# OliBomby/Mapperatorinator

Measured on NVIDIA H100. Metric: event tokens/sec end-to-end (mel+T5+DiT), higher is better.
Workload: dtype f32

## Files before the change

mapperatorinator_b200/csrc/attention.cu:

```cuda
#include "common.cuh"
#include "kernels.h"

namespace mb200 {
namespace {

constexpr int TQ = 64, TK = 64, HD = 64, LDS_ = 68;

__device__ __forceinline__ bool mask_allowed(const AttentionParams& p, int b, int q, int k) {
    if (k >= p.Tk) return false;
    if (p.key_valid && !p.key_valid[(long long)b * p.key_valid_ld + k]) return false;
    switch (p.mask_mode) {
        case MASK_CAUSAL: return k <= p.q_pos0 + q;
        case MASK_BAND:   return (q >= k - p.band) && (q < k + p.band);
        case MASK_DENSE:  return q < p.Tq && !p.dense[(long long)q * p.Tk + k];
        default:          return true;
    }
}

__global__ void __launch_bounds__(256) attention_kernel(AttentionParams p) {
    extern __shared__ __align__(16) float smem[];
    float (*Qt)[LDS_] = reinterpret_cast<float (*)[LDS_]>(smem);
    float (*Kt)[LDS_] = reinterpret_cast<float (*)[LDS_]>(smem + HD * LDS_);
    float (*Vs)[LDS_] = reinterpret_cast<float (*)[LDS_]>(smem + 2 * HD * LDS_);
    float (*Ps)[LDS_] = reinterpret_cast<float (*)[LDS_]>(smem + 3 * HD * LDS_);

    const int tid = threadIdx.x, tx = tid & 15, ty = tid >> 4;
    const int q0 = blockIdx.x * TQ, h = blockIdx.y, b = blockIdx.z;
    const float* qb = p.q + (long long)b * p.q_bs + h * HD;
    const int kvb = p.kv_slot ? p.kv_slot[b] : b;
    const float* kb = p.k + (long long)kvb * p.k_bs + h * HD;
    const float* vb = p.v + (long long)kvb * p.v_bs + h * HD;

    {
        const int r = tid >> 4, dq = (tid & 15) * 4;
#pragma unroll
        for (int rr = 0; rr < 4; ++rr) {
            int row = r + rr * 16, q = q0 + row;
            float4 v = q < p.Tq ? *reinterpret_cast<const float4*>(qb + (long long)q * p.q_ld + dq) : make_float4(0, 0, 0, 0);
            Qt[dq + 0][row] = v.x * p.scale; Qt[dq + 1][row] = v.y * p.scale;
            Qt[dq + 2][row] = v.z * p.scale; Qt[dq + 3][row] = v.w * p.scale;
        }
    }

    int kt_begin = 0, kt_end = (p.Tk + TK - 1) / TK;
    if (p.mask_mode == MASK_CAUSAL) {
        int last = p.q_pos0 + min(q0 + TQ - 1, p.Tq - 1);
        kt_end = min(kt_end, last / TK + 1);
    } else if (p.mask_mode == MASK_BAND) {
        int lo = q0 - p.band + 1, hi = min(q0 + TQ - 1, p.Tq - 1) + p.band;
        kt_begin = max(0, lo) / TK;
        kt_end = min(kt_end, hi / TK + 1);
    }

    float m_i[4], l_i[4], o[4][4];
#pragma unroll
    for (int i = 0; i < 4; ++i) {
        m_i[i] = -INFINITY; l_i[i] = 0.f;
#pragma unroll
        for (int j = 0; j < 4; ++j) o[i][j] = 0.f;
    }

    for (int kt = kt_begin; kt < kt_end; ++kt) {
        const int k0 = kt * TK;
        __syncthreads();
        {
            const int r = tid >> 4, dq = (tid & 15) * 4;
#pragma unroll
            for (int rr = 0; rr < 4; ++rr) {
                int row = r + rr * 16, k = k0 + row;
                float4 kv = make_float4(0, 0, 0, 0), vv = make_float4(0, 0, 0, 0);
                if (k < p.Tk) {
                    kv = *reinterpret_cast<const float4*>(kb + (long long)k * p.k_ld + dq);
                    vv = *reinterpret_cast<const float4*>(vb + (long long)k * p.v_ld + dq);
                }
                Kt[dq + 0][row] = kv.x; Kt[dq + 1][row] = kv.y; Kt[dq + 2][row] = kv.z; Kt[dq + 3][row] = kv.w;
                *reinterpret_cast<float4*>(&Vs[row][dq]) = vv;
            }
        }
        __syncthreads();

        float s[4][4];
#pragma unroll
        for (int i = 0; i < 4; ++i)
#pragma unroll
            for (int j = 0; j < 4; ++j) s[i][j] = 0.f;
#pragma unroll 16
        for (int d = 0; d < HD; ++d) {
            float4 qa = *reinterpret_cast<const float4*>(&Qt[d][ty * 4]);
            float4 ka = *reinterpret_cast<const float4*>(&Kt[d][tx * 4]);
            float qv[4] = {qa.x, qa.y, qa.z, qa.w}, kv[4] = {ka.x, ka.y, ka.z, ka.w};
#pragma unroll
            for (int i = 0; i < 4; ++i)
#pragma unroll
                for (int j = 0; j < 4; ++j) s[i][j] = fmaf(qv[i], kv[j], s[i][j]);
        }

#pragma unroll
        for (int i = 0; i < 4; ++i) {
            const int q = q0 + ty * 4 + i;
            float mx = -INFINITY;
#pragma unroll
            for (int j = 0; j < 4; ++j) {
                if (!mask_allowed(p, b, q, k0 + tx * 4 + j)) s[i][j] = -INFINITY;
                mx = fmaxf(mx, s[i][j]);
            }
#pragma unroll
            for (int off = 8; off > 0; off >>= 1) mx = fmaxf(mx, __shfl_xor_sync(0xffffffffu, mx, off));
            const float m_new = fmaxf(m_i[i], mx);
            const float corr = (m_new == -INFINITY) ? 1.f : expf(m_i[i] - m_new);
            float psum = 0.f;
            float pr[4];
#pragma unroll
            for (int j = 0; j < 4; ++j) {
                pr[j] = (s[i][j] == -INFINITY) ? 0.f : expf(s[i][j] - m_new);
                psum += pr[j];
            }
            l_i[i] = l_i[i] * corr + psum;
            m_i[i] = m_new;
#pragma unroll
            for (int j = 0; j < 4; ++j) o[i][j] *= corr;
            *reinterpret_cast<float4*>(&Ps[ty * 4 + i][tx * 4]) = make_float4(pr[0], pr[1], pr[2], pr[3]);
        }
        __syncthreads();

#pragma unroll 4
        for (int c4 = 0; c4 < TK / 4; ++c4) {
            float4 pa[4], va[4];
#pragma unroll
            for (int i = 0; i < 4; ++i) pa[i] = *reinterpret_cast<const float4*>(&Ps[ty * 4 + i][c4 * 4]);
#pragma unroll
            for (int c = 0; c < 4; ++c) va[c] = *reinterpret_cast<const float4*>(&Vs[c4 * 4 + c][tx * 4]);
#pragma unroll
            for (int i = 0; i < 4; ++i) {
                const float pv[4] = {pa[i].x, pa[i].y, pa[i].z, pa[i].w};
#pragma unroll
                for (int c = 0; c < 4; ++c) {
                    o[i][0] = fmaf(pv[c], va[c].x, o[i][0]); o[i][1] = fmaf(pv[c], va[c].y, o[i][1]);
                    o[i][2] = fmaf(pv[c], va[c].z, o[i][2]); o[i][3] = fmaf(pv[c], va[c].w, o[i][3]);
                }
            }
        }
    }

    float* ob = p.o + (long long)b * p.o_bs + h * HD;
#pragma unroll
    for (int i = 0; i < 4; ++i) {
        float l = l_i[i];
#pragma unroll
        for (int off = 8; off > 0; off >>= 1) l += __shfl_xor_sync(0xffffffffu, l, off);
        const int q = q0 + ty * 4 + i;
        if (q >= p.Tq) continue;
        const float inv = l > 0.f ? 1.0f / l : 0.f;
        *reinterpret_cast<float4*>(ob + (long long)q * p.o_ld + tx * 4) =
            make_float4(o[i][0] * inv, o[i][1] * inv, o[i][2] * inv, o[i][3] * inv);
    }
}

}

int launch_attention(const AttentionParams& p, cudaStream_t stream, AttnCtx* ctx) {
    MB_REQUIRE(p.q_ld % 4 == 0 && p.k_ld % 4 == 0 && p.v_ld % 4 == 0 && p.o_ld % 4 == 0, "attention strides must be multiples of 4");
    if (p.B <= 0 || p.Tq <= 0) return 0;
    if (attn_tc_eligible(p, ctx)) return launch_attention_tc(p, stream, ctx);
    static bool configured = false;
    const int smem_bytes = 4 * HD * LDS_ * (int)sizeof(float);
    if (!configured) {
        MB_CUDA_CHECK(cudaFuncSetAttribute(attention_kernel, cudaFuncAttributeMaxDynamicSharedMemorySize, smem_bytes));
        configured = true;
    }
    dim3 grid((p.Tq + TQ - 1) / TQ, p.H, p.B);
    attention_kernel<<<grid, 256, smem_bytes, stream>>>(p);
    MB_LAUNCH_CHECK();
    ++g_launch_count;
    return 0;
}

}
```

mapperatorinator_b200/csrc/engine_model.cu:

```cuda
#include <algorithm>
#include <cstring>
#include <map>
#include <tuple>
#include <unordered_map>
#include <vector>

#include "../../include/mapperatorinator_b200.h"
#include "common.cuh"
#include "kernels.h"

using namespace mb200;

namespace {

struct DevBuf {
    void* p = nullptr;
    size_t bytes = 0;
    int ensure(size_t need, bool zero = false) {
        if (need <= bytes) return 0;
        if (p) cudaFree(p);
        p = nullptr; bytes = 0;
        MB_CUDA_CHECK(cudaMalloc(&p, need));
        bytes = need;
        if (zero) MB_CUDA_CHECK(cudaMemset(p, 0, need));
        return 0;
    }
    template <typename T> T* as() const { return reinterpret_cast<T*>(p); }
    ~DevBuf() { if (p) cudaFree(p); }
};

struct LayerW {
    const float *ln1_w, *ln1_b, *wqkv, *bqkv, *wo, *bo;
    const float *ln2_w, *ln2_b, *wq_c, *bq_c, *wkv_c, *bkv_c, *wo_c, *bo_c;
    const float *ln3_w, *ln3_b, *fc1_w, *fc1_b, *fc2_w, *fc2_b;
};

}

struct mb200_model {
    mb200_model_config cfg;
    MelPlan* mel = nullptr;
    std::unordered_map<std::string, std::vector<float>> host_w;
    bool finalized = false;

    DevBuf arena;
    const float *emb_w = nullptr, *emb_b = nullptr, *conv1_w = nullptr, *conv1_b = nullptr, *conv2_w = nullptr, *conv2_b = nullptr,
                *enc_pos = nullptr, *enc_ln_w = nullptr, *enc_ln_b = nullptr;
    const float *tok_emb = nullptr, *dec_pos = nullptr, *dec_ln_w = nullptr, *dec_ln_b = nullptr, *proj_out = nullptr;
    std::vector<LayerW> enc, dec;

    DevBuf cross_kv;
    DevBuf self_kv;
    int max_rows = 0;

    int enc_chunk = 0;
    DevBuf w_mel, w_embpad, w_c1pad, w_x, w_h, w_qkv, w_attn, w_ffn;
    DevBuf p_x, p_h, p_q, p_attn, p_ffn;
    DevBuf d_x, d_q, d_h, d_parto, d_partml, d_logits;
    DevBuf d_attn, d_ticket;
    DevBuf g_state, g_cfg, g_vflags, g_ids, g_prefill_ids, g_keyvalid, g_leftpad, g_rowslot, g_finished, g_lastts, g_lastscores;
    int* h_flag = nullptr;
    std::map<std::tuple<int, int, int, int>, cudaGraphExec_t> graphs;
    std::map<std::tuple<int, int, int, int>, long long> graph_nodes;
    bool use_pdl = false;
    cudaStream_t cap_stream = nullptr;
    std::map<std::tuple<int, int, int, int>, int> prefill_seen;
    std::map<std::tuple<int, int, int, int>, std::pair<cudaGraphExec_t, long long>> prefill_graphs;
    int enc_graph = 1;
    int trace_cta = 0;
    int use_mega = 2;
    DevBuf ll_arena;
    MegaLL ll{};
    size_t ll_bytes = 0;
    std::map<std::tuple<int, int, int>, std::pair<DevBuf*, int>> mega2_phases;
    int num_sms = 0;
    int num_sms_phys = 0;
    DevBuf g_megasync;
    DevBuf mega_trace;
    cudaEvent_t mega_ev[2] = {nullptr, nullptr};
    double mega_ms = 0.0; long long mega_launches = 0, mega_tokens = 0;
    std::map<std::pair<int, int>, std::pair<DevBuf*, int>> mega_phases;
    DevBuf w_pcm;
    std::map<int, std::pair<cudaGraphExec_t, long long>> enc_graphs;
    std::map<int, int> enc_seen;
    DevBuf b_kvsrc, b_logprobs, b_cand, b_runscore, b_finids[2], b_finscore, b_finlen, b_finflag, b_unsat;
    DevBuf b_dbg;
    AttnCtx attn;
    GemmCtx gemm;

    int d() const { return cfg.d_model; }
    int Ts() const { return cfg.src_seq_len / 2; }
    size_t cross_layer_stride() const { return (size_t)cfg.max_windows * Ts() * 2 * d(); }
    size_t self_layer_stride() const { return (size_t)max_rows * cfg.tgt_seq_len * 2 * d(); }
};

namespace {

std::vector<std::string> required_names(const mb200_model_config& c) {
    std::vector<std::string> n = {
        "encoder_embedder.weight", "encoder_embedder.bias", "decoder_embedder.weight",
        "transformer.model.encoder.conv1.weight", "transformer.model.encoder.conv1.bias",
        "transformer.model.encoder.conv2.weight", "transformer.model.encoder.conv2.bias",
        "transformer.model.encoder.embed_positions.weight",
        "transformer.model.encoder.layer_norm.weight", "transformer.model.encoder.layer_norm.bias",
        "transformer.model.decoder.embed_positions.weight",
        "transformer.model.decoder.layer_norm.weight", "transformer.model.decoder.layer_norm.bias",
        "transformer.proj_out.weight"};
    auto attn = [&](const std::string& p) {
        n.push_back(p + "q_proj.weight"); n.push_back(p + "q_proj.bias"); n.push_back(p + "k_proj.weight");
        n.push_back(p + "v_proj.weight"); n.push_back(p + "v_proj.bias");
        n.push_back(p + "out_proj.weight"); n.push_back(p + "out_proj.bias");
    };
    auto ln = [&](const std::string& p) { n.push_back(p + "weight"); n.push_back(p + "bias"); };
    for (int side = 0; side < 2; ++side) {
        int L = side == 0 ? c.encoder_layers : c.decoder_layers;
        for (int i = 0; i < L; ++i) {
            std::string p = std::string("transformer.model.") + (side == 0 ? "encoder" : "decoder") + ".layers." + std::to_string(i) + ".";
            attn(p + "self_attn."); ln(p + "self_attn_layer_norm.");
            if (side == 1) { attn(p + "encoder_attn."); ln(p + "encoder_attn_layer_norm."); }
            n.push_back(p + "fc1.weight"); n.push_back(p + "fc1.bias"); n.push_back(p + "fc2.weight"); n.push_back(p + "fc2.bias");
            ln(p + "final_layer_norm.");
        }
    }
    return n;
}

GemmParams gemm_base(const RowMap& A, const float* W, long long ldw, const RowMap& C, const float* bias, int M, int N, int K) {
    GemmParams g{};
    g.A = A; g.W = W; g.ldw = ldw; g.C = C; g.bias = bias; g.act = ACT_NONE; g.alpha = 1.f;
    g.gate = nullptr; g.gate_ld = 0; g.gate_rpb = 1; g.R = RowMap{nullptr, 0, 0, 0};
    g.M = M; g.N = N; g.K = K;
    return g;
}

#define MB_TRY(expr) do { int _s = (expr); if (_s) return _s; } while (0)

int layernorm(const float* x, float* y, const float* w, const float* b, int rows, int dim, float eps, cudaStream_t st) {
    LayerNormParams p{};
    p.x = x; p.ldx = dim; p.y = y; p.ldy = dim; p.weight = w; p.bias = b; p.shift = nullptr; p.scale = nullptr; p.mod_ld = 0;
    p.rows_per_batch = 1; p.rows = rows; p.dim = dim; p.eps = eps;
    return launch_layernorm(p, st);
}

}

extern "C" int mb200_model_create(mb200_model** out, const mb200_model_config* cfg, const float* mel_basis_host) {
    MB_REQUIRE(cfg && out, "null argument");
    MB_REQUIRE(cfg->d_model == cfg->heads * 64, "kernels are specialised for head_dim 64 (whisper-small: 768 / 12)");
    MB_REQUIRE(cfg->d_model % 128 == 0 && cfg->d_model <= 1024, "d_model must be a multiple of 128 and <= 1024");
    MB_REQUIRE(cfg->vocab_size_out <= 4096, "fused sampling kernel holds the vocabulary in shared memory (<= 4096 ids)");
    MB_REQUIRE(cfg->mel.n_mels % 4 == 0 && cfg->ffn_dim % 4 == 0, "n_mels / ffn_dim must be multiples of 4");
    mb200_model* m = new mb200_model();
    m->cfg = *cfg;
    int s = mel_plan_create(&m->mel, cfg->mel.n_fft, cfg->mel.hop_length, cfg->mel.n_mels, cfg->mel.pad_reflect, cfg->mel.log_scale,
                            mel_basis_host);
    if (s) { delete m; return s; }
    if (cudaMallocHost(&m->h_flag, 64) != cudaSuccess) { delete m; set_last_error("cudaMallocHost failed"); return 1; }
    {
        int dev = 0, coop = 0;
        cudaGetDevice(&dev);
        cudaDeviceGetAttribute(&m->num_sms, cudaDevAttrMultiProcessorCount, dev);
        m->num_sms_phys = m->num_sms;
        cudaDeviceGetAttribute(&coop, cudaDevAttrCooperativeLaunch, dev);
        if (!coop) m->num_sms = 0;
    }
    *out = m;
    return 0;
}

extern "C" void mb200_model_destroy(mb200_model* m) {
    if (!m) return;
    for (auto& g : m->graphs) cudaGraphExecDestroy(g.second);
    for (auto& g : m->prefill_graphs) cudaGraphExecDestroy(g.second.first);
    for (auto& g : m->enc_graphs) cudaGraphExecDestroy(g.second.first);
    m->gemm.destroy();
    m->attn.destroy();
    for (auto& kv : m->mega_phases) delete kv.second.first;
    for (auto& kv : m->mega2_phases) delete kv.second.first;
    for (auto& e : m->mega_ev) if (e) cudaEventDestroy(e);
    if (m->cap_stream) cudaStreamDestroy(m->cap_stream);
    mel_plan_destroy(m->mel);
    if (m->h_flag) cudaFreeHost(m->h_flag);
    delete m;
}

extern "C" int mb200_model_set_weight(mb200_model* m, const char* name, const float* data, int64_t numel) {
    MB_REQUIRE(m && name && data, "null argument");
    MB_REQUIRE(!m->finalized, "model already finalized");
    m->host_w[name] = std::vector<float>(data, data + numel);
    return 0;
}

extern "C" int mb200_model_finalize(mb200_model* m) {
    MB_REQUIRE(m && !m->finalized, "bad model state");
    const auto& c = m->cfg;
    const int d = c.d_model, f = c.ffn_dim;
    for (const auto& n : required_names(c))
        MB_REQUIRE(m->host_w.count(n) == 1, std::string("missing weight ") + n);
    auto W = [&](const std::string& n) -> const std::vector<float>& { return m->host_w.at(n); };
    auto expect = [&](const std::string& n, size_t numel) -> int {
        MB_REQUIRE(W(n).size() == numel, "wrong element count for " + n);
        return 0;
    };
    MB_TRY(expect("encoder_embedder.weight", (size_t)d * c.mel.n_mels));
    MB_TRY(expect("decoder_embedder.weight", (size_t)c.vocab_size_in * d));
    MB_TRY(expect("transformer.proj_out.weight", (size_t)c.vocab_size_out * d));
    MB_TRY(expect("transformer.model.encoder.conv1.weight", (size_t)d * d * 3));
    MB_TRY(expect("transformer.model.encoder.embed_positions.weight", (size_t)(c.src_seq_len / 2) * d));
    MB_TRY(expect("transformer.model.decoder.embed_positions.weight", (size_t)c.tgt_seq_len * d));

    std::vector<float> pack;
    auto push = [&](const std::vector<float>& v) -> size_t {
        size_t off = (pack.size() + 63) & ~size_t(63);
        pack.resize(off + v.size());
        std::copy(v.begin(), v.end(), pack.begin() + off);
        return off;
    };
    auto conv_pack = [&](const std::vector<float>& w) {
        std::vector<float> o((size_t)d * 3 * d);
        for (int co = 0; co < d; ++co)
            for (int ci = 0; ci < d; ++ci)
                for (int j = 0; j < 3; ++j) o[(size_t)co * 3 * d + (size_t)j * d + ci] = w[((size_t)co * d + ci) * 3 + j];
        return o;
    };
    const float qs = 0.125f;
    auto qkv_pack = [&](const std::string& p, std::vector<float>& wq, std::vector<float>& bq) {
        wq.assign((size_t)3 * d * d, 0.f); bq.assign((size_t)3 * d, 0.f);
        const auto &q = W(p + "q_proj.weight"), &k = W(p + "k_proj.weight"), &v = W(p + "v_proj.weight");
        const auto &qb = W(p + "q_proj.bias"), &vb = W(p + "v_proj.bias");
        for (size_t i = 0; i < (size_t)d * d; ++i) { wq[i] = q[i] * qs; wq[(size_t)d * d + i] = k[i]; wq[(size_t)2 * d * d + i] = v[i]; }
        for (int i = 0; i < d; ++i) { bq[i] = qb[i] * qs; bq[2 * d + i] = vb[i]; }
    };
    struct Off { size_t v[20]; };
    std::vector<Off> eo(c.encoder_layers), dof(c.decoder_layers);
    size_t o_emb_w = push(W("encoder_embedder.weight")), o_emb_b = push(W("encoder_embedder.bias"));
    size_t o_c1w = push(conv_pack(W("transformer.model.encoder.conv1.weight"))), o_c1b = push(W("transformer.model.encoder.conv1.bias"));
    size_t o_c2w = push(conv_pack(W("transformer.model.encoder.conv2.weight"))), o_c2b = push(W("transformer.model.encoder.conv2.bias"));
    size_t o_epos = push(W("transformer.model.encoder.embed_positions.weight"));
    size_t o_elnw = push(W("transformer.model.encoder.layer_norm.weight")), o_elnb = push(W("transformer.model.encoder.layer_norm.bias"));
    size_t o_tok = push(W("decoder_embedder.weight")), o_dpos = push(W("transformer.model.decoder.embed_positions.weight"));
    size_t o_dlnw = push(W("transformer.model.decoder.layer_norm.weight")), o_dlnb = push(W("transformer.model.decoder.layer_norm.bias"));
    size_t o_proj = push(W("transformer.proj_out.weight"));
    for (int side = 0; side < 2; ++side) {
        int L = side == 0 ? c.encoder_layers : c.decoder_layers;
        for (int i = 0; i < L; ++i) {
            std::string p = std::string("transformer.model.") + (side == 0 ? "encoder" : "decoder") + ".layers." + std::to_string(i) + ".";
            Off& o = side == 0 ? eo[i] : dof[i];
            std::vector<float> wq, bq;
            qkv_pack(p + "self_attn.", wq, bq);
            o.v[0] = push(W(p + "self_attn_layer_norm.weight")); o.v[1] = push(W(p + "self_attn_layer_norm.bias"));
            o.v[2] = push(wq); o.v[3] = push(bq);
            o.v[4] = push(W(p + "self_attn.out_proj.weight")); o.v[5] = push(W(p + "self_attn.out_proj.bias"));
            if (side == 1) {
                qkv_pack(p + "encoder_attn.", wq, bq);
                o.v[6] = push(W(p + "encoder_attn_layer_norm.weight")); o.v[7] = push(W(p + "encoder_attn_layer_norm.bias"));
                o.v[8] = push(std::vector<float>(wq.begin(), wq.begin() + (size_t)d * d));
                o.v[9] = push(std::vector<float>(bq.begin(), bq.begin() + d));
                o.v[10] = push(std::vector<float>(wq.begin() + (size_t)d * d, wq.end()));
                o.v[11] = push(std::vector<float>(bq.begin() + d, bq.end()));
                o.v[12] = push(W(p + "encoder_attn.out_proj.weight")); o.v[13] = push(W(p + "encoder_attn.out_proj.bias"));
            }
            o.v[14] = push(W(p + "final_layer_norm.weight")); o.v[15] = push(W(p + "final_layer_norm.bias"));
            o.v[16] = push(W(p + "fc1.weight")); o.v[17] = push(W(p + "fc1.bias"));
            o.v[18] = push(W(p + "fc2.weight")); o.v[19] = push(W(p + "fc2.bias"));
            MB_REQUIRE(W(p + "fc1.weight").size() == (size_t)f * d, "wrong fc1 shape");
        }
    }
    MB_TRY(m->arena.ensure(pack.size() * sizeof(float)));
    MB_CUDA_CHECK(cudaMemcpy(m->arena.p, pack.data(), pack.size() * sizeof(float), cudaMemcpyHostToDevice));
    const float* base = m->arena.as<float>();
    m->emb_w = base + o_emb_w; m->emb_b = base + o_emb_b; m->conv1_w = base + o_c1w; m->conv1_b = base + o_c1b;
    m->conv2_w = base + o_c2w; m->conv2_b = base + o_c2b; m->enc_pos = base + o_epos; m->enc_ln_w = base + o_elnw; m->enc_ln_b = base + o_elnb;
    m->tok_emb = base + o_tok; m->dec_pos = base + o_dpos; m->dec_ln_w = base + o_dlnw; m->dec_ln_b = base + o_dlnb; m->proj_out = base + o_proj;
    auto fill = [&](const Off& o, bool cross) {
        LayerW l{};
        l.ln1_w = base + o.v[0]; l.ln1_b = base + o.v[1]; l.wqkv = base + o.v[2]; l.bqkv = base + o.v[3]; l.wo = base + o.v[4]; l.bo = base + o.v[5];
        if (cross) {
            l.ln2_w = base + o.v[6]; l.ln2_b = base + o.v[7]; l.wq_c = base + o.v[8]; l.bq_c = base + o.v[9];
            l.wkv_c = base + o.v[10]; l.bkv_c = base + o.v[11]; l.wo_c = base + o.v[12]; l.bo_c = base + o.v[13];
        }
        l.ln3_w = base + o.v[14]; l.ln3_b = base + o.v[15]; l.fc1_w = base + o.v[16]; l.fc1_b = base + o.v[17];
        l.fc2_w = base + o.v[18]; l.fc2_b = base + o.v[19];
        return l;
    };
    for (auto& o : eo) m->enc.push_back(fill(o, false));
    for (auto& o : dof) m->dec.push_back(fill(o, true));
    m->host_w.clear();
    {
        const long long dd = (long long)d * d;
        auto reg = [&](const float* w, long long n) -> int { return m->gemm.register_weight(w, n); };
        MB_TRY(reg(m->emb_w, (long long)d * c.mel.n_mels));
        MB_TRY(reg(m->conv1_w, 3 * dd)); MB_TRY(reg(m->conv2_w, 3 * dd));
        for (const auto& l : m->enc) {
            MB_TRY(reg(l.wqkv, 3 * dd)); MB_TRY(reg(l.wo, dd));
            MB_TRY(reg(l.fc1_w, (long long)f * d)); MB_TRY(reg(l.fc2_w, (long long)f * d));
        }
        for (const auto& l : m->dec) MB_TRY(reg(l.wkv_c, 2 * dd));
        MB_CUDA_CHECK(cudaDeviceSynchronize());
        const size_t chunk = (size_t)std::min(std::max(1, c.max_windows), 16);
        const size_t a_floats = std::max({chunk * (size_t)(c.src_seq_len / 2) * f, chunk * (size_t)(c.src_seq_len + 2) * d,
                                          chunk * (size_t)c.src_seq_len * c.mel.n_mels});
        m->gemm.num_sms = std::max(1, m->num_sms_phys);
        MB_TRY(m->gemm.reserve((size_t)64 << 20, a_floats * 8 + 1024));
        m->gemm.frozen = true;
        MB_TRY(m->attn.reserve(attn_tc_workspace_bytes((int)chunk, c.heads, c.src_seq_len / 2, c.src_seq_len / 2)));
        m->attn.frozen = true;
    }

    m->max_rows = std::max(1, c.max_batch);
    MB_TRY(m->cross_kv.ensure((size_t)c.decoder_layers * m->cross_layer_stride() * sizeof(float)));
    MB_TRY(m->self_kv.ensure((size_t)c.decoder_layers * m->self_layer_stride() * sizeof(float)));
    MB_TRY(m->g_state.ensure(sizeof(GenState) + (size_t)m->max_rows * sizeof(RowState)));
    MB_TRY(m->g_cfg.ensure((size_t)m->max_rows * sizeof(SampleConfig)));
    MB_TRY(m->g_vflags.ensure((size_t)m->max_rows * c.vocab_size_in));
    MB_TRY(m->g_ids.ensure((size_t)m->max_rows * c.tgt_seq_len * sizeof(long long)));
    MB_TRY(m->g_prefill_ids.ensure((size_t)m->max_rows * c.tgt_seq_len * sizeof(long long)));
    MB_TRY(m->g_keyvalid.ensure((size_t)m->max_rows * c.tgt_seq_len));
    MB_TRY(m->g_leftpad.ensure(m->max_rows * sizeof(int)));
    MB_TRY(m->g_rowslot.ensure((size_t)3 * m->max_rows * sizeof(int)));
    MB_TRY(m->g_finished.ensure(m->max_rows));
    MB_TRY(m->g_lastts.ensure(m->max_rows * sizeof(int)));
    MB_TRY(m->g_lastscores.ensure((size_t)2 * m->max_rows * c.vocab_size_out * sizeof(float)));
    MB_TRY(m->d_x.ensure((size_t)m->max_rows * d * sizeof(float)));
    MB_TRY(m->d_q.ensure((size_t)m->max_rows * d * sizeof(float)));
    MB_TRY(m->d_h.ensure((size_t)m->max_rows * f * sizeof(float)));
    MB_TRY(m->d_logits.ensure((size_t)m->max_rows * c.vocab_size_out * sizeof(float)));
    {
        const size_t RPmax = (size_t)m->max_rows * c.tgt_seq_len;
        MB_TRY(m->p_x.ensure(RPmax * d * 4)); MB_TRY(m->p_h.ensure(RPmax * d * 4)); MB_TRY(m->p_q.ensure(RPmax * d * 4));
        MB_TRY(m->p_attn.ensure(RPmax * d * 4)); MB_TRY(m->p_ffn.ensure(RPmax * f * 4));
    }
    {
        const int max_splits = std::max((c.tgt_seq_len + 63) / 64, (c.src_seq_len / 2 + 63) / 64);
        MB_TRY(m->d_parto.ensure((size_t)m->max_rows * c.heads * max_splits * 64 * sizeof(float)));
        MB_TRY(m->d_partml.ensure((size_t)m->max_rows * c.heads * max_splits * 2 * sizeof(float)));
        MB_TRY(m->d_attn.ensure((size_t)m->max_rows * d * sizeof(float)));
        MB_TRY(m->d_ticket.ensure((size_t)m->max_rows * c.heads * sizeof(int)));
        MB_CUDA_CHECK(cudaMemset(m->d_ticket.p, 0, (size_t)m->max_rows * c.heads * sizeof(int)));
    }
    {
        const int R2 = 2, max_splits = std::max((c.tgt_seq_len + 63) / 64, (c.src_seq_len / 2 + 63) / 64);
        auto al = [](size_t n) { return (n + 15) & ~size_t(15); };
        const size_t n_x = al((size_t)R2 * d), n_kv = al((size_t)R2 * 2 * d), n_h = al((size_t)R2 * f), n_l = al((size_t)R2 * c.vocab_size_out),
                     n_p = al((size_t)R2 * c.heads * max_splits * 66), n_hdr = 16;
        const size_t RM = MEGA_LL_MAX_REPS;
        m->ll_bytes = ((2 * RM + 1) * n_x + n_kv + RM * n_h + n_l + n_p + n_hdr) * 8;
        MB_TRY(m->ll_arena.ensure(m->ll_bytes, true));
        unsigned long long* b = m->ll_arena.as<unsigned long long>();
        m->ll.x = b; b += RM * n_x; m->ll.att = b; b += RM * n_x; m->ll.q = b; b += n_x; m->ll.kvnew = b; b += n_kv; m->ll.h = b; b += RM * n_h;
        m->ll.logits = b; b += n_l; m->ll.part = b; b += n_p; m->ll.hdr = b;
        m->ll.max_splits = max_splits;
        m->ll.reps = 8; m->ll.x_rep = (long long)n_x; m->ll.h_rep = (long long)n_h;
    }
    m->finalized = true;
    return 0;
}

static int encode_chunk(mb200_model* m, const float* pcm, int n, int slot_begin, float* enc_out, cudaStream_t st) {
    const auto& c = m->cfg;
    const int d = c.d_model, f = c.ffn_dim, H = c.heads, T2 = c.src_seq_len, T = T2 / 2, nm = c.mel.n_mels;
    const int n_samples = (c.src_seq_len - 1) * c.mel.hop_length;
    float* mel = m->w_mel.as<float>();
    float* embp = m->w_embpad.as<float>();
    float* c1p = m->w_c1pad.as<float>();
    float* x = m->w_x.as<float>();
    float* h = m->w_h.as<float>();
    float* qkv = m->w_qkv.as<float>();
    float* att = m->w_attn.as<float>();
    float* ffn = m->w_ffn.as<float>();
    const long long padrow = (long long)(T2 + 2) * d;

    MB_TRY(launch_mel(m->mel, pcm, n_samples, n, n_samples, mel, nm, (long long)T2 * nm, st));
    {
        GemmParams g = gemm_base(plain_map(mel, nm), m->emb_w, nm, batched_map(embp + d, d, T2, padrow), m->emb_b, n * T2, d, nm);
        MB_TRY(launch_gemm(g, st, &m->gemm));
    }
    {
        GemmParams g = gemm_base(batched_map(embp, d, T2, padrow), m->conv1_w, 3 * d, batched_map(c1p + d, d, T2, padrow), m->conv1_b,
                                 n * T2, d, 3 * d);
        g.act = ACT_GELU_ERF;
        MB_TRY(launch_gemm(g, st, &m->gemm));
    }
    {
        GemmParams g = gemm_base(batched_map(c1p, 2 * d, T, padrow), m->conv2_w, 3 * d, plain_map(x, d), m->conv2_b, n * T, d, 3 * d);
        g.act = ACT_GELU_ERF;
        g.R = batched_map(m->enc_pos, d, T, 0);
        MB_TRY(launch_gemm(g, st, &m->gemm));
    }
    const int rows = n * T;
    for (int l = 0; l < c.encoder_layers; ++l) {
        const LayerW& w = m->enc[l];
        MB_TRY(layernorm(x, h, w.ln1_w, w.ln1_b, rows, d, 1e-5f, st));
        MB_TRY(launch_gemm(gemm_base(plain_map(h, d), w.wqkv, d, plain_map(qkv, 3 * d), w.bqkv, rows, 3 * d, d), st, &m->gemm));
        AttentionParams a{};
        a.q = qkv; a.q_ld = 3 * d; a.q_bs = (long long)T * 3 * d;
        a.k = qkv + d; a.k_ld = 3 * d; a.k_bs = a.q_bs;
        a.v = qkv + 2 * d; a.v_ld = 3 * d; a.v_bs = a.q_bs;
        a.o = att; a.o_ld = d; a.o_bs = (long long)T * d;
        a.B = n; a.H = H; a.Tq = T; a.Tk = T; a.scale = 1.f; a.mask_mode = MASK_NONE;
        MB_TRY(launch_attention(a, st, &m->attn));
        {
            GemmParams g = gemm_base(plain_map(att, d), w.wo, d, plain_map(x, d), w.bo, rows, d, d);
            g.R = plain_map(x, d);
            MB_TRY(launch_gemm(g, st, &m->gemm));
        }
        MB_TRY(layernorm(x, h, w.ln3_w, w.ln3_b, rows, d, 1e-5f, st));
        {
            GemmParams g = gemm_base(plain_map(h, d), w.fc1_w, d, plain_map(ffn, f), w.fc1_b, rows, f, d);
            g.act = ACT_GELU_ERF;
            MB_TRY(launch_gemm(g, st, &m->gemm));
        }
        {
            GemmParams g = gemm_base(plain_map(ffn, f), w.fc2_w, f, plain_map(x, d), w.fc2_b, rows, d, f);
            g.R = plain_map(x, d);
            MB_TRY(launch_gemm(g, st, &m->gemm));
        }
    }
    float* enc = enc_out ? enc_out : h;
    MB_TRY(layernorm(x, enc, m->enc_ln_w, m->enc_ln_b, rows, d, 1e-5f, st));
    for (int l = 0; l < c.decoder_layers; ++l) {
        float* dst = m->cross_kv.as<float>() + (size_t)l * m->cross_layer_stride() + (size_t)slot_begin * T * 2 * d;
        MB_TRY(launch_gemm(gemm_base(plain_map(enc, d), m->dec[l].wkv_c, d, plain_map(dst, 2 * d), m->dec[l].bkv_c, rows, 2 * d, d), st, &m->gemm));
    }
    return 0;
}

extern "C" int mb200_model_encode(mb200_model* m, const float* pcm, int32_t n_windows, int32_t slot_begin, float* enc_out, void* stream) {
    MB_REQUIRE(m && m->finalized, "model not finalized");
    MB_REQUIRE(slot_begin >= 0 && slot_begin + n_windows <= m->cfg.max_windows, "encoder slots out of range (raise max_windows)");
    cudaStream_t st = (cudaStream_t)stream;
    const auto& c = m->cfg;
    const int d = c.d_model, T2 = c.src_seq_len, T = T2 / 2;
    const int chunk = std::min(n_windows, 16);
    if (chunk > m->enc_chunk) {
        MB_TRY(m->w_mel.ensure((size_t)chunk * T2 * c.mel.n_mels * 4));
        MB_TRY(m->w_embpad.ensure((size_t)chunk * (T2 + 2) * d * 4, true));
        MB_TRY(m->w_c1pad.ensure((size_t)chunk * (T2 + 2) * d * 4, true));
        MB_TRY(m->w_x.ensure((size_t)chunk * T * d * 4));
        MB_TRY(m->w_h.ensure((size_t)chunk * T * d * 4));
        MB_TRY(m->w_qkv.ensure((size_t)chunk * T * 3 * d * 4));
        MB_TRY(m->w_attn.ensure((size_t)chunk * T * d * 4));
        MB_TRY(m->w_ffn.ensure((size_t)chunk * T * c.ffn_dim * 4));
        m->enc_chunk = chunk;
        for (auto& g : m->enc_graphs) cudaGraphExecDestroy(g.second.first);
        m->enc_graphs.clear(); m->enc_seen.clear();
    }
    const long long n_samples = (long long)(c.src_seq_len - 1) * c.mel.hop_length;
    if (n_windows == 1 && enc_out == nullptr && m->enc_graph) {
        auto seen = m->enc_seen.find(slot_begin);
        if (seen == m->enc_seen.end()) {
            m->enc_seen[slot_begin] = 1;
            return encode_chunk(m, pcm, 1, slot_begin, nullptr, st);
        }
        MB_TRY(m->w_pcm.ensure((size_t)n_samples * sizeof(float)));
        auto git = m->enc_graphs.find(slot_begin);
        if (git == m->enc_graphs.end()) {
            if (!m->cap_stream) MB_CUDA_CHECK(cudaStreamCreateWithFlags(&m->cap_stream, cudaStreamNonBlocking));
            MB_CUDA_CHECK(cudaStreamSynchronize(st));
            cudaGraph_t graph;
            MB_CUDA_CHECK(cudaStreamBeginCapture(m->cap_stream, cudaStreamCaptureModeThreadLocal));
            const long long before = g_launch_count;
            int rc = encode_chunk(m, m->w_pcm.as<float>(), 1, slot_begin, nullptr, m->cap_stream);
            cudaError_t e = cudaStreamEndCapture(m->cap_stream, &graph);
            const long long nodes = g_launch_count - before;
            g_launch_count = before;
            if (rc) return rc;
            MB_CUDA_CHECK(e);
            cudaGraphExec_t exec;
            MB_CUDA_CHECK(cudaGraphInstantiate(&exec, graph, 0));
            cudaGraphDestroy(graph);
            git = m->enc_graphs.emplace(slot_begin, std::make_pair(exec, nodes)).first;
        }
        MB_CUDA_CHECK(cudaMemcpyAsync(m->w_pcm.p, pcm, (size_t)n_samples * sizeof(float), cudaMemcpyDeviceToDevice, st));
        MB_CUDA_CHECK(cudaGraphLaunch(git->second.first, st));
        g_launch_count += git->second.second;
        return 0;
    }
    for (int i = 0; i < n_windows; i += m->enc_chunk) {
        int n = std::min(m->enc_chunk, n_windows - i);
        MB_TRY(encode_chunk(m, pcm + (long long)i * n_samples, n, slot_begin + i, enc_out ? enc_out + (long long)i * T * d : nullptr, st));
    }
    return 0;
}

static int decoder_prefill(mb200_model* m, int rows, int P, const long long* ids_dev, int pos_rule, cudaStream_t st, int cache_row0 = 0,
                           int cache_row_step = 1, const int* row_slot = nullptr) {
    const auto& c = m->cfg;
    const int d = c.d_model, f = c.ffn_dim, H = c.heads, T = c.src_seq_len / 2;
    const size_t RP = (size_t)rows * P;
    MB_TRY(m->p_x.ensure(RP * d * 4)); MB_TRY(m->p_h.ensure(RP * d * 4)); MB_TRY(m->p_q.ensure(RP * d * 4));
    MB_TRY(m->p_attn.ensure(RP * d * 4)); MB_TRY(m->p_ffn.ensure(RP * f * 4));
    float *x = m->p_x.as<float>(), *h = m->p_h.as<float>(), *q = m->p_q.as<float>(), *att = m->p_attn.as<float>(), *ffn = m->p_ffn.as<float>();
    const unsigned char* kv_valid = m->g_keyvalid.as<unsigned char>();
    if (!row_slot) row_slot = m->g_rowslot.as<int>();
    MB_TRY(launch_embed(ids_dev, P, rows, rows, P, m->g_leftpad.as<int>(), pos_rule, m->tok_emb, m->dec_pos, d, x, st));
    const long long self_row = (long long)c.tgt_seq_len * 2 * d * cache_row_step;
    for (int l = 0; l < c.decoder_layers; ++l) {
        const LayerW& w = m->dec[l];
        float* skv = m->self_kv.as<float>() + (size_t)l * m->self_layer_stride() + (size_t)cache_row0 * c.tgt_seq_len * 2 * d;
        const float* ckv = m->cross_kv.as<float>() + (size_t)l * m->cross_layer_stride();
        MB_TRY(layernorm(x, h, w.ln1_w, w.ln1_b, (int)RP, d, 1e-5f, st));
        MB_TRY(launch_gemm(gemm_base(plain_map(h, d), w.wqkv, d, plain_map(q, d), w.bqkv, (int)RP, d, d), st, &m->gemm));
        MB_TRY(launch_gemm(gemm_base(plain_map(h, d), w.wqkv + (size_t)d * d, d, batched_map(skv, 2 * d, P, self_row), w.bqkv + d, (int)RP,
                                     2 * d, d), st, &m->gemm));
        AttentionParams a{};
        a.q = q; a.q_ld = d; a.q_bs = (long long)P * d;
        a.k = skv; a.k_ld = 2 * d; a.k_bs = self_row;
        a.v = skv + d; a.v_ld = 2 * d; a.v_bs = self_row;
        a.o = att; a.o_ld = d; a.o_bs = (long long)P * d;
        a.B = rows; a.H = H; a.Tq = P; a.Tk = P; a.scale = 1.f; a.mask_mode = MASK_CAUSAL; a.q_pos0 = 0;
        a.key_valid = kv_valid; a.key_valid_ld = c.tgt_seq_len;
        MB_TRY(launch_attention(a, st));
        {
            GemmParams g = gemm_base(plain_map(att, d), w.wo, d, plain_map(x, d), w.bo, (int)RP, d, d);
            g.R = plain_map(x, d);
            MB_TRY(launch_gemm(g, st, &m->gemm));
        }
        MB_TRY(layernorm(x, h, w.ln2_w, w.ln2_b, (int)RP, d, 1e-5f, st));
        MB_TRY(launch_gemm(gemm_base(plain_map(h, d), w.wq_c, d, plain_map(q, d), w.bq_c, (int)RP, d, d), st, &m->gemm));
        AttentionParams ca{};
        ca.q = q; ca.q_ld = d; ca.q_bs = (long long)P * d;
        ca.k = ckv; ca.k_ld = 2 * d; ca.k_bs = (long long)T * 2 * d;
        ca.v = ckv + d; ca.v_ld = 2 * d; ca.v_bs = ca.k_bs;
        ca.o = att; ca.o_ld = d; ca.o_bs = (long long)P * d;
        ca.B = rows; ca.H = H; ca.Tq = P; ca.Tk = T; ca.scale = 1.f; ca.mask_mode = MASK_NONE; ca.kv_slot = row_slot;
        MB_TRY(launch_attention(ca, st));
        {
            GemmParams g = gemm_base(plain_map(att, d), w.wo_c, d, plain_map(x, d), w.bo_c, (int)RP, d, d);
            g.R = plain_map(x, d);
            MB_TRY(launch_gemm(g, st, &m->gemm));
        }
        MB_TRY(layernorm(x, h, w.ln3_w, w.ln3_b, (int)RP, d, 1e-5f, st));
        {
            GemmParams g = gemm_base(plain_map(h, d), w.fc1_w, d, plain_map(ffn, f), w.fc1_b, (int)RP, f, d);
            g.act = ACT_GELU_ERF;
            MB_TRY(launch_gemm(g, st, &m->gemm));
        }
        {
            GemmParams g = gemm_base(plain_map(ffn, f), w.fc2_w, f, plain_map(x, d), w.fc2_b, (int)RP, d, f);
            g.R = plain_map(x, d);
            MB_TRY(launch_gemm(g, st, &m->gemm));
        }
    }
    return 0;
}

static GemvParams gemv_base(int xmode, const float* W, long long ldw, const float* bias, int K, int N, int B, const GenState* stt) {
    GemvParams g{};
    g.xmode = xmode; g.W = W; g.ldw = ldw; g.bias = bias; g.K = K; g.N = N; g.B = B; g.st = stt; g.eps = 1e-5f; g.nseg = 1;
    g.seg[0] = GemvSeg{nullptr, 0, 0, 0, N, 1.f, ACT_NONE};
    return g;
}

static GemvParams final_logits_params(mb200_model* m, int rows, const float* x, long long x_ld) {
    const auto& c = m->cfg;
    GemvParams g = gemv_base(X_LAYERNORM, m->proj_out, c.d_model, nullptr, c.d_model, c.vocab_size_out, rows, m->g_state.as<GenState>());
    g.x = x; g.x_ld = x_ld; g.ln_w = m->dec_ln_w; g.ln_b = m->dec_ln_b;
    g.seg[0].out = m->d_logits.as<float>(); g.seg[0].out_bs = c.vocab_size_out;
    return g;
}

static int final_logits(mb200_model* m, int rows, const float* x, long long x_ld, cudaStream_t st, bool pdl) {
    return launch_gemv(final_logits_params(m, rows, x, x_ld), st, pdl);
}

static SampleParams sample_params(mb200_model* m, int rows) {
    const auto& c = m->cfg;
    SampleParams s{};
    s.logits = m->d_logits.as<float>(); s.logits_ld = c.vocab_size_out;
    s.cfg = m->g_cfg.as<SampleConfig>(); s.st = m->g_state.as<GenState>(); s.vflags = m->g_vflags.as<unsigned char>();
    s.ids = m->g_ids.as<long long>(); s.finished = m->g_finished.as<unsigned char>(); s.last_ts = m->g_lastts.as<int>();
    s.last_scores = m->g_lastscores.as<float>(); s.n_left_pad = m->g_leftpad.as<int>();
    s.tok_emb = m->tok_emb; s.pos_emb = m->dec_pos; s.d_model = c.d_model;
    s.x_out = m->d_x.as<float>(); s.x_ld = c.d_model; s.rows = rows;
    return s;
}

static int token_step(mb200_model* m, int rows, int B, int n_splits_self, cudaStream_t st, bool pdl,
                      std::vector<MegaPhase>* collect = nullptr, const BeamParams* beam = nullptr, bool ragged = false) {
    auto emit_gemv = [&](const GemvParams& g) -> int {
        if (!collect) return launch_gemv(g, st, pdl, ragged && g.nseg > 1);
        MegaPhase ph{}; ph.kind = 0; ph.g = g; collect->push_back(ph);
        return 0;
    };
    auto emit_attn = [&](const DecAttnParams& a) -> int {
        if (!collect) return launch_decode_attention(a, st, pdl);
        MegaPhase ph{}; ph.kind = 1; ph.a = a;
        ph.magic_ns = a.n_splits > 1 ? (unsigned)((1ull << 32) / (unsigned)a.n_splits + 1) : 0u;
        ph.magic_h = a.H > 1 ? (unsigned)((1ull << 32) / (unsigned)a.H + 1) : 0u;
        collect->push_back(ph);
        return 0;
    };
    const auto& c = m->cfg;
    const int d = c.d_model, f = c.ffn_dim, H = c.heads, T = c.src_seq_len / 2;
    const GenState* gs = m->g_state.as<GenState>();
    float *x = m->d_x.as<float>(), *q = m->d_q.as<float>(), *hh = m->d_h.as<float>();
    float *po = m->d_parto.as<float>(), *pml = m->d_partml.as<float>(), *attn = m->d_attn.as<float>();
    int* ticket = m->d_ticket.as<int>();
    const int chunk = 64, n_splits_cross = (T + chunk - 1) / chunk;
    const long long self_row = (long long)c.tgt_seq_len * 2 * d;
    for (int l = 0; l < c.decoder_layers; ++l) {
        const LayerW& w = m->dec[l];
        float* skv = m->self_kv.as<float>() + (size_t)l * m->self_layer_stride();
        const float* ckv = m->cross_kv.as<float>() + (size_t)l * m->cross_layer_stride();
        {
            GemvParams g = gemv_base(X_LAYERNORM, w.wqkv, d, w.bqkv, d, 3 * d, rows, gs);
            g.x = x; g.x_ld = d; g.ln_w = w.ln1_w; g.ln_b = w.ln1_b;
            g.nseg = 3;
            g.seg[0] = GemvSeg{q, d, 0, 0, d, 1.f, ACT_NONE};
            g.seg[1] = GemvSeg{skv, self_row, 2 * d, d, 2 * d, 1.f, ACT_NONE};
            g.seg[2] = GemvSeg{skv + d, self_row, 2 * d, 2 * d, 3 * d, 1.f, ACT_NONE};
            MB_TRY(emit_gemv(g));
        }
        {
            DecAttnParams a{};
            a.q = q; a.q_ld = d; a.kc = skv; a.vc = skv + d; a.row_stride = self_row; a.tok_stride = 2 * d; a.row_slot = nullptr;
            a.fixed_len = 0; a.st = gs; a.key_valid = m->g_keyvalid.as<unsigned char>(); a.key_valid_ld = c.tgt_seq_len;
            a.part_o = po; a.part_ml = pml; a.rows = rows; a.H = H; a.n_splits = n_splits_self;
            a.chunk = n_splits_self == 1 ? 128 : chunk;
            a.out = attn; a.out_ld = d; a.ticket = ticket;
            if (beam) { a.kv_src = beam->kv_src; a.kv_src_ld = beam->kv_src_ld; }
            if (ragged) {
                a.key_valid = nullptr;
                MB_TRY(launch_decode_attention_ragged(a, st, pdl));
            } else
            MB_TRY(emit_attn(a));
        }
        {
            GemvParams g = gemv_base(X_PLAIN, w.wo, d, w.bo, d, d, rows, gs);
            g.x = attn; g.x_ld = d;
            g.seg[0].out = x; g.seg[0].out_bs = d; g.R = x; g.r_ld = d;
            MB_TRY(emit_gemv(g));
        }
        {
            GemvParams g = gemv_base(X_LAYERNORM, w.wq_c, d, w.bq_c, d, d, rows, gs);
            g.x = x; g.x_ld = d; g.ln_w = w.ln2_w; g.ln_b = w.ln2_b;
            g.seg[0].out = q; g.seg[0].out_bs = d;
            MB_TRY(emit_gemv(g));
        }
        {
            DecAttnParams a{};
            a.q = q; a.q_ld = d; a.kc = ckv; a.vc = ckv + d; a.row_stride = (long long)T * 2 * d; a.tok_stride = 2 * d;
            a.row_slot = m->g_rowslot.as<int>(); a.fixed_len = T; a.st = gs; a.key_valid = nullptr;
            a.part_o = po; a.part_ml = pml; a.rows = rows; a.H = H; a.n_splits = n_splits_cross; a.chunk = chunk;
            a.out = attn; a.out_ld = d; a.ticket = ticket;
            MB_TRY(emit_attn(a));
        }
        {
            GemvParams g = gemv_base(X_PLAIN, w.wo_c, d, w.bo_c, d, d, rows, gs);
            g.x = attn; g.x_ld = d;
            g.seg[0].out = x; g.seg[0].out_bs = d; g.R = x; g.r_ld = d;
            MB_TRY(emit_gemv(g));
        }
        {
            GemvParams g = gemv_base(X_LAYERNORM, w.fc1_w, d, w.fc1_b, d, f, rows, gs);
            g.x = x; g.x_ld = d; g.ln_w = w.ln3_w; g.ln_b = w.ln3_b;
            g.seg[0] = GemvSeg{hh, f, 0, 0, f, 1.f, ACT_GELU_ERF};
            MB_TRY(emit_gemv(g));
        }
        {
            GemvParams g = gemv_base(X_PLAIN, w.fc2_w, f, w.fc2_b, f, d, rows, gs);
            g.x = hh; g.x_ld = f;
            g.seg[0].out = x; g.seg[0].out_bs = d; g.R = x; g.r_ld = d;
            MB_TRY(emit_gemv(g));
        }
    }
    MB_TRY(emit_gemv(final_logits_params(m, rows, x, d)));
    if (collect) {
        MegaPhase ph{}; ph.kind = 2; collect->push_back(ph);
        const int n = (int)collect->size();
        for (int i = 0; i < n; ++i) {
            int j = (i + 1) % n;
            while ((*collect)[j].kind != 0) j = (j + 1) % n;
            (*collect)[i].next_gemv = j;
            (*collect)[i].nx_W = (*collect)[j].g.W; (*collect)[i].nx_ldw = (*collect)[j].g.ldw;
            (*collect)[i].nx_N = (*collect)[j].g.N; (*collect)[i].nx_K = (*collect)[j].g.K;
            (*collect)[i].nx_rpc = ((*collect)[j].g.N + m->num_sms - 1) / m->num_sms;
            (*collect)[i].rpc = (*collect)[i].kind == 0 ? ((*collect)[i].g.N + m->num_sms - 1) / m->num_sms : 0;
        }
        return 0;
    }
    if (beam) return launch_beam_step(*beam, B, st);
    MB_TRY(launch_sample(sample_params(m, rows), B, st, pdl, ragged));
    return 0;
}

static int run_megakernel(mb200_model* m, int rows, int B, int n_splits_self, int max_steps, cudaStream_t st) {
    auto key = std::make_pair(rows, n_splits_self);
    auto it = m->mega_phases.find(key);
    if (it == m->mega_phases.end()) {
        std::vector<MegaPhase> phases;
        MB_TRY(token_step(m, rows, B, n_splits_self, st, false, &phases));
        DevBuf* buf = new DevBuf();
        MB_TRY(buf->ensure(phases.size() * sizeof(MegaPhase)));
        MB_CUDA_CHECK(cudaMemcpy(buf->p, phases.data(), phases.size() * sizeof(MegaPhase), cudaMemcpyHostToDevice));
        it = m->mega_phases.emplace(key, std::make_pair(buf, (int)phases.size())).first;
    }
    MB_TRY(m->g_megasync.ensure(64));
    MB_CUDA_CHECK(cudaMemsetAsync(m->g_megasync.p, 0, 64, st));
    MegaParams mp{};
    mp.phases = it->second.first->as<MegaPhase>(); mp.n_phases = it->second.second; mp.first_gemv = 0;
    mp.sample = sample_params(m, rows); mp.st = m->g_state.as<GenState>();
    mp.sync_counter = m->g_megasync.as<unsigned int>(); mp.error_flag = m->g_megasync.as<int>() + 8;
    mp.max_steps = max_steps; mp.row_slot = m->g_rowslot.as<int>();
    mp.trace = m->mega_trace.p ? m->mega_trace.as<unsigned long long>() : nullptr; mp.trace_step = 8;
    if (!m->mega_ev[0]) { MB_CUDA_CHECK(cudaEventCreate(&m->mega_ev[0])); MB_CUDA_CHECK(cudaEventCreate(&m->mega_ev[1])); }
    MB_CUDA_CHECK(cudaMemcpyAsync(m->h_flag + 2, &m->g_state.as<GenState>()->cur_len, 4, cudaMemcpyDeviceToHost, st));
    MB_CUDA_CHECK(cudaEventRecord(m->mega_ev[0], st));
    MB_TRY(launch_megakernel(mp, m->num_sms, st));
    MB_CUDA_CHECK(cudaEventRecord(m->mega_ev[1], st));
    MB_CUDA_CHECK(cudaMemcpyAsync(m->h_flag + 1, m->g_megasync.as<int>() + 8, 4, cudaMemcpyDeviceToHost, st));
    MB_CUDA_CHECK(cudaMemcpyAsync(m->h_flag + 3, &m->g_state.as<GenState>()->cur_len, 4, cudaMemcpyDeviceToHost, st));
    MB_CUDA_CHECK(cudaStreamSynchronize(st));
    {
        float ms = 0.f;
        MB_CUDA_CHECK(cudaEventElapsedTime(&ms, m->mega_ev[0], m->mega_ev[1]));
        m->mega_ms += ms; m->mega_launches += 1; m->mega_tokens += m->h_flag[3] - m->h_flag[2];
    }
    MB_REQUIRE(m->h_flag[1] == 0, m->h_flag[1] == 1 ? "megakernel grid barrier timed out" : "megakernel weight copy timed out");
    return 0;
}

static int run_megakernel2(mb200_model* m, int rows, int B, int n_splits_self, int max_steps, cudaStream_t st) {
    auto key = std::make_tuple(rows, B, n_splits_self);
    auto it = m->mega2_phases.find(key);
    if (it == m->mega2_phases.end()) {
        std::vector<MegaPhase> phases;
        MB_TRY(token_step(m, rows, B, n_splits_self, st, false, &phases));
        std::vector<Mega2Phase> p2(phases.size());
        const float *dx = m->d_x.as<float>(), *dq = m->d_q.as<float>(), *dh = m->d_h.as<float>(), *datt = m->d_attn.as<float>(),
                    *dlog = m->d_logits.as<float>();
        for (size_t i = 0; i < phases.size(); ++i) {
            Mega2Phase& q = p2[i];
            q = Mega2Phase{};
            q.base = phases[i];
            if (phases[i].kind != 0) continue;
            const GemvParams& g = phases[i].g;
            q.in_sel = g.xmode == X_LAYERNORM ? LL_X : (g.x == datt ? LL_ATT : (g.x == dh ? LL_H : LL_NONE));
            MB_REQUIRE(q.in_sel != LL_NONE && (g.xmode != X_LAYERNORM || g.x == dx), "dataflow megakernel: unknown GEMV input buffer");
            q.res_xraw = g.R != nullptr;
            MB_REQUIRE(!g.R || g.R == dx, "dataflow megakernel: residual must be the residual stream");
            for (int sgi = 0; sgi < g.nseg; ++sgi) {
                const GemvSeg& sg = g.seg[sgi];
                if (sg.pos_stride != 0) { q.out_sel[sgi] = sgi == 1 ? LL_K : LL_V; q.plain_out[sgi] = 1; MB_REQUIRE(sgi >= 1, "cache segment order"); }
                else if (sg.out == dq) q.out_sel[sgi] = LL_Q;
                else if (sg.out == dx) q.out_sel[sgi] = LL_X;
                else if (sg.out == dh) q.out_sel[sgi] = LL_H;
                else if (sg.out == dlog) q.out_sel[sgi] = LL_LOGITS;
                else MB_REQUIRE(false, "dataflow megakernel: unknown GEMV output buffer");
                const int os = q.out_sel[sgi];
                const unsigned long long* ob = os == LL_X ? m->ll.x : os == LL_H ? m->ll.h : os == LL_Q ? m->ll.q : os == LL_LOGITS ? m->ll.logits : m->ll.kvnew;
                q.out_off[sgi] = (long long)(ob - m->ll.x) + (os == LL_V ? m->cfg.d_model : 0);
                q.out_rs[sgi] = os == LL_X ? m->ll.x_rep : (os == LL_H ? m->ll.h_rep : 0);
                q.out_bw[sgi] = os == LL_H ? g.N : (os == LL_K || os == LL_V ? 2 * m->cfg.d_model : (os == LL_LOGITS ? m->cfg.vocab_size_out : m->cfg.d_model));
            }
            {
                const unsigned long long* ib = q.in_sel == LL_H ? m->ll.h : (q.in_sel == LL_ATT ? m->ll.att : m->ll.x);
                q.in_off = (long long)(ib - m->ll.x);
                q.in_rs = q.in_sel == LL_H ? m->ll.h_rep : m->ll.x_rep;
                const int rpc = (g.N + m->num_sms - 1) / m->num_sms;
                q.n_active = (g.N + rpc - 1) / rpc;
            }
        }
        DevBuf* buf = new DevBuf();
        MB_TRY(buf->ensure(p2.size() * sizeof(Mega2Phase)));
        MB_CUDA_CHECK(cudaMemcpy(buf->p, p2.data(), p2.size() * sizeof(Mega2Phase), cudaMemcpyHostToDevice));
        it = m->mega2_phases.emplace(key, std::make_pair(buf, (int)p2.size())).first;
    }
    MB_TRY(m->g_megasync.ensure(64));
    MB_CUDA_CHECK(cudaMemsetAsync(m->g_megasync.p, 0, 64, st));
    MB_CUDA_CHECK(cudaMemsetAsync(m->ll_arena.p, 0, m->ll_bytes, st));
    Mega2Params mp{};
    mp.phases = it->second.first->as<Mega2Phase>(); mp.n_phases = it->second.second;
    mp.sample = sample_params(m, rows); mp.st = m->g_state.as<GenState>();
    mp.ll = m->ll; mp.error_flag = m->g_megasync.as<int>() + 8;
    mp.sample.ll_logits = m->ll.logits; mp.sample.ll_x_out = m->ll.x; mp.sample.ll_hdr = m->ll.hdr; mp.sample.ll_err = mp.error_flag;
    mp.sample.ll_reps = m->ll.reps; mp.sample.ll_x_rep = m->ll.x_rep;
    mp.max_steps = max_steps; mp.row_slot = m->g_rowslot.as<int>(); mp.x_in = m->d_x.as<float>();
    mp.rows = rows; mp.d_model = m->cfg.d_model; mp.V = m->cfg.vocab_size_out; mp.ffn_dim = m->cfg.ffn_dim; mp.trace_cta = m->trace_cta;
    mp.trace = m->mega_trace.p ? m->mega_trace.as<unsigned long long>() : nullptr; mp.trace_step = 8;
    if (!m->mega_ev[0]) { MB_CUDA_CHECK(cudaEventCreate(&m->mega_ev[0])); MB_CUDA_CHECK(cudaEventCreate(&m->mega_ev[1])); }
    MB_CUDA_CHECK(cudaMemcpyAsync(m->h_flag + 2, &m->g_state.as<GenState>()->cur_len, 4, cudaMemcpyDeviceToHost, st));
    MB_CUDA_CHECK(cudaEventRecord(m->mega_ev[0], st));
    MB_TRY(launch_megakernel2(mp, m->num_sms, st));
    MB_CUDA_CHECK(cudaEventRecord(m->mega_ev[1], st));
    MB_CUDA_CHECK(cudaMemcpyAsync(m->h_flag + 1, m->g_megasync.as<int>() + 8, 4, cudaMemcpyDeviceToHost, st));
    MB_CUDA_CHECK(cudaMemcpyAsync(m->h_flag + 3, &m->g_state.as<GenState>()->cur_len, 4, cudaMemcpyDeviceToHost, st));
    MB_CUDA_CHECK(cudaStreamSynchronize(st));
    {
        float ms = 0.f;
        MB_CUDA_CHECK(cudaEventElapsedTime(&ms, m->mega_ev[0], m->mega_ev[1]));
        m->mega_ms += ms; m->mega_launches += 1; m->mega_tokens += m->h_flag[3] - m->h_flag[2];
    }
    MB_REQUIRE(m->h_flag[1] == 0, m->h_flag[1] == 2 ? "dataflow megakernel: weight copy timed out" : "dataflow megakernel: a wait for tagged data timed out");
    return 0;
}

static bool mega_eligible(const mb200_model* m, int rows) {
    if (!m->use_mega || rows > 2 || m->num_sms <= 0) return false;
    const auto& c = m->cfg;
    const int G = m->num_sms;
    auto slice = [&](int N, int K) { return (size_t)((N + G - 1) / G) * K; };
    const int d = c.d_model, f = c.ffn_dim;
    const size_t qkv = slice(3 * d, d), dd = slice(d, d), fc1 = slice(f, d), fc2 = slice(d, f), voc = slice(c.vocab_size_out, d);
    auto pair = [&](size_t a, size_t b) { return a + b <= (size_t)2 * MEGA_WBUF_FLOATS; };
    return f <= 3072 && pair(qkv, dd) && pair(dd, dd) && pair(dd, fc1) && pair(fc1, fc2) && pair(fc2, qkv) && pair(fc2, voc) && pair(voc, qkv);
}

static SampleConfig make_sample_config(const mb200_generate_params* gp, int B, bool use_cfg, int V, int ids_ld) {
    SampleConfig sc{};
    sc.B = B; sc.use_cfg = use_cfg ? 1 : 0; sc.cfg_scale = gp->cfg_scale; sc.V = V; sc.ts_start = gp->time_shift_start; sc.ts_end = gp->time_shift_end;
    sc.timeshift_bias = gp->timeshift_bias; sc.types_first = gp->types_first; sc.temperature = gp->temperature;
    sc.n_cond = gp->n_cond;
    for (int i = 0; i < 3; ++i) { sc.cond_temp[i] = gp->cond_temp[i]; sc.cond_offset[i] = gp->cond_offset[i]; sc.cond_flag[i] = gp->cond_flag[i]; }
    sc.lookback_on = gp->lookback_on; sc.lookback_start = gp->lookback_start; sc.lookback_end = gp->lookback_end;
    sc.do_sample = gp->do_sample; sc.top_k = gp->top_k; sc.top_p = gp->top_p; sc.top_p_cut = gp->top_p_cut; sc.seed = gp->seed; sc.pad_id = gp->pad_token_id;
    sc.pos_rule_cumsum = gp->position_rule; sc.ids_ld = ids_ld; sc.vflags_ld = 0;
    return sc;
}

extern "C" int mb200_model_generate(mb200_model* m, const int32_t* slots, int32_t B, const int64_t* prompt, const uint8_t* prompt_mask,
                                    int32_t P, const int64_t* neg_prompt, const uint8_t* neg_mask, const uint8_t* vflags,
                                    const mb200_generate_params* gp, int64_t* out_ids, int32_t* out_len, void* stream) {
    MB_REQUIRE(m && m->finalized, "model not finalized");
    MB_REQUIRE(slots && prompt && vflags && gp && out_ids && out_len, "null argument");
    const auto& c = m->cfg;
    cudaStream_t st = (cudaStream_t)stream;
    const bool use_cfg = neg_prompt != nullptr;
    const int rows = use_cfg ? 2 * B : B;
    MB_REQUIRE(B >= 1 && rows <= m->max_rows, "batch exceeds max_batch (rows double under classifier-free guidance)");
    MB_REQUIRE(P >= 1 && P < gp->max_length && gp->max_length <= c.tgt_seq_len, "need 1 <= prompt_len < max_length <= tgt_seq_len");
    for (int b = 0; b < B; ++b) MB_REQUIRE(slots[b] >= 0 && slots[b] < c.max_windows, "encoder slot out of range");
    const int d = c.d_model, H = c.heads, T = c.src_seq_len / 2, V = c.vocab_size_out;
    const int ids_ld = c.tgt_seq_len;

    std::vector<long long> pre((size_t)rows * P), idsrow((size_t)B * ids_ld, (long long)gp->pad_token_id);
    std::vector<unsigned char> kv((size_t)rows * ids_ld, 1);
    std::vector<int> leftpad(rows, 0), rowslot(rows);
    for (int r = 0; r < rows; ++r) {
        const int b = r % B;
        const bool neg_row = use_cfg && r < B;
        const int64_t* src = neg_row ? neg_prompt : prompt;
        const uint8_t* msk = neg_row ? (neg_mask ? neg_mask : prompt_mask) : prompt_mask;
        int npad = 0; bool seen = false;
        for (int t = 0; t < P; ++t) {
            long long tok = src[(size_t)b * P + t];
            MB_REQUIRE(tok >= 0 && tok < c.vocab_size_in, "prompt token id out of range");
            pre[(size_t)r * P + t] = tok;
            unsigned char ok = msk ? (msk[(size_t)b * P + t] != 0) : 1;
            kv[(size_t)r * ids_ld + t] = ok;
            if (!ok && !seen) ++npad; else seen = true;
        }
        leftpad[r] = npad;
        rowslot[r] = slots[b];
    }
    for (int b = 0; b < B; ++b)
        for (int t = 0; t < P; ++t) idsrow[(size_t)b * ids_ld + t] = prompt[(size_t)b * P + t];
    GenState gs{};
    gs.cur_len = P; gs.prompt_len = P; gs.max_length = gp->max_length; gs.min_new_tokens = gp->min_new_tokens;
    const SampleConfig sc = make_sample_config(gp, B, use_cfg, V, ids_ld);

    MB_CUDA_CHECK(cudaMemcpyAsync(m->g_prefill_ids.p, pre.data(), pre.size() * 8, cudaMemcpyHostToDevice, st));
    MB_CUDA_CHECK(cudaMemcpyAsync(m->g_ids.p, idsrow.data(), idsrow.size() * 8, cudaMemcpyHostToDevice, st));
    MB_CUDA_CHECK(cudaMemcpyAsync(m->g_keyvalid.p, kv.data(), kv.size(), cudaMemcpyHostToDevice, st));
    MB_CUDA_CHECK(cudaMemcpyAsync(m->g_leftpad.p, leftpad.data(), rows * 4, cudaMemcpyHostToDevice, st));
    MB_CUDA_CHECK(cudaMemcpyAsync(m->g_rowslot.p, rowslot.data(), rows * 4, cudaMemcpyHostToDevice, st));
    MB_CUDA_CHECK(cudaMemcpyAsync(m->g_vflags.p, vflags, c.vocab_size_in, cudaMemcpyHostToDevice, st));
    MB_CUDA_CHECK(cudaMemcpyAsync(m->g_state.p, &gs, sizeof(gs), cudaMemcpyHostToDevice, st));
    MB_CUDA_CHECK(cudaMemcpyAsync(m->g_cfg.p, &sc, sizeof(sc), cudaMemcpyHostToDevice, st));
    MB_CUDA_CHECK(cudaMemsetAsync(m->g_finished.p, 0, m->max_rows, st));
    MB_CUDA_CHECK(cudaMemsetAsync(m->d_ticket.p, 0, (size_t)m->max_rows * m->cfg.heads * sizeof(int), st));
    MB_CUDA_CHECK(cudaStreamSynchronize(st));

    const int chunk = 64;
    const int n_splits_self = self_splits(gp->max_length);
    (void)H; (void)T;

    MB_TRY(launch_prompt_scan(m->g_ids.as<long long>(), ids_ld, B, P, m->g_vflags.as<unsigned char>(), sc.ts_start, sc.ts_end,
                              m->g_lastts.as<int>(), st));
    {
        auto run_prefill = [&](cudaStream_t s) -> int {
            MB_TRY(decoder_prefill(m, rows, P, m->g_prefill_ids.as<long long>(), gp->position_rule, s));
            MB_TRY(final_logits(m, rows, m->p_x.as<float>() + (size_t)(P - 1) * d, (long long)P * d, s, false));
            MB_TRY(launch_sample(sample_params(m, rows), B, s, false));
            return 0;
        };
        const auto pkey = std::make_tuple(rows, (int)B, (int)P, (int)gp->position_rule);
        auto seen = m->prefill_seen.find(pkey);
        if (seen == m->prefill_seen.end()) {
            m->prefill_seen[pkey] = 1;
            MB_TRY(run_prefill(st));
        } else {
            auto git = m->prefill_graphs.find(pkey);
            if (git == m->prefill_graphs.end()) {
                if (!m->cap_stream) MB_CUDA_CHECK(cudaStreamCreateWithFlags(&m->cap_stream, cudaStreamNonBlocking));
                MB_CUDA_CHECK(cudaStreamSynchronize(st));
                cudaGraph_t graph;
                MB_CUDA_CHECK(cudaStreamBeginCapture(m->cap_stream, cudaStreamCaptureModeThreadLocal));
                const long long before = g_launch_count;
                int s = run_prefill(m->cap_stream);
                cudaError_t e = cudaStreamEndCapture(m->cap_stream, &graph);
                const long long nodes = g_launch_count - before;
                g_launch_count = before;
                if (s) return s;
                MB_CUDA_CHECK(e);
                cudaGraphExec_t exec;
                MB_CUDA_CHECK(cudaGraphInstantiate(&exec, graph, 0));
                cudaGraphDestroy(graph);
                if (m->prefill_graphs.size() >= 48) {
                    for (auto& g : m->prefill_graphs) cudaGraphExecDestroy(g.second.first);
                    m->prefill_graphs.clear();
                    m->prefill_seen.clear();
                }
                git = m->prefill_graphs.emplace(pkey, std::make_pair(exec, nodes)).first;
            }
            MB_CUDA_CHECK(cudaGraphLaunch(git->second.first, st));
            g_launch_count += git->second.second;
        }
    }

    if (mega_eligible(m, rows) && gp->max_length - (P + 1) > 0) {
        bool dataflow = m->use_mega >= 2;
        if (dataflow) {
            const int G = m->num_sms;
            dataflow = mega2_ksplit_ok(3 * c.d_model, c.d_model, rows, G) && mega2_ksplit_ok(c.d_model, c.d_model, rows, G) &&
                       mega2_ksplit_ok(c.ffn_dim, c.d_model, rows, G) && mega2_ksplit_ok(c.d_model, c.ffn_dim, rows, G) &&
                       mega2_ksplit_ok(c.vocab_size_out, c.d_model, rows, G);
        }
        if (dataflow) MB_TRY(run_megakernel2(m, rows, B, n_splits_self, gp->max_length - (P + 1), st));
        else MB_TRY(run_megakernel(m, rows, B, n_splits_self, gp->max_length - (P + 1), st));
        MB_CUDA_CHECK(cudaMemcpyAsync(m->h_flag, &m->g_state.as<GenState>()->cur_len, 4, cudaMemcpyDeviceToHost, st));
        MB_CUDA_CHECK(cudaStreamSynchronize(st));
        const int Lm = *m->h_flag;
        MB_CUDA_CHECK(cudaMemcpy2DAsync(out_ids, (size_t)Lm * 8, m->g_ids.p, (size_t)ids_ld * 8, (size_t)Lm * 8, B, cudaMemcpyDeviceToHost, st));
        MB_CUDA_CHECK(cudaStreamSynchronize(st));
        *out_len = Lm;
        return 0;
    }
    auto key = std::make_tuple(rows, (int)B, n_splits_self, 1);
    auto it = m->graphs.find(key);
    if (it == m->graphs.end()) {
        cudaGraph_t graph;
        if (!m->cap_stream) MB_CUDA_CHECK(cudaStreamCreateWithFlags(&m->cap_stream, cudaStreamNonBlocking));
        MB_CUDA_CHECK(cudaStreamSynchronize(st));
        MB_CUDA_CHECK(cudaStreamBeginCapture(m->cap_stream, cudaStreamCaptureModeThreadLocal));
        const long long before = g_launch_count;
        int s = token_step(m, rows, B, n_splits_self, m->cap_stream, m->use_pdl);
        cudaError_t e = cudaStreamEndCapture(m->cap_stream, &graph);
        m->graph_nodes[key] = g_launch_count - before;
        g_launch_count = before;
        if (s) return s;
        MB_CUDA_CHECK(e);
        cudaGraphExec_t exec;
        MB_CUDA_CHECK(cudaGraphInstantiate(&exec, graph, 0));
        cudaGraphDestroy(graph);
        it = m->graphs.emplace(key, exec).first;
    }
    int remaining = gp->max_length - (P + 1);
    const int burst_default = 16;
    int produced = 1;
    while (remaining > 0) {
        int burst = std::min(remaining, burst_default);
        if (gp->min_new_tokens > produced) burst = std::min(remaining, std::max(burst, gp->min_new_tokens - produced));
        for (int i = 0; i < burst; ++i) MB_CUDA_CHECK(cudaGraphLaunch(it->second, st));
        g_launch_count += (long long)burst * m->graph_nodes[key];
        remaining -= burst; produced += burst;
        MB_CUDA_CHECK(cudaMemcpyAsync(m->h_flag, &m->g_state.as<GenState>()->all_finished, 4, cudaMemcpyDeviceToHost, st));
        MB_CUDA_CHECK(cudaStreamSynchronize(st));
        if (*m->h_flag) break;
    }
    MB_CUDA_CHECK(cudaMemcpyAsync(m->h_flag, &m->g_state.as<GenState>()->cur_len, 4, cudaMemcpyDeviceToHost, st));
    MB_CUDA_CHECK(cudaStreamSynchronize(st));
    const int L = *m->h_flag;
    MB_CUDA_CHECK(cudaMemcpy2DAsync(out_ids, (size_t)L * 8, m->g_ids.p, (size_t)ids_ld * 8, (size_t)L * 8, B, cudaMemcpyDeviceToHost, st));
    MB_CUDA_CHECK(cudaStreamSynchronize(st));
    *out_len = L;
    return 0;
}

extern "C" int mb200_model_generate_ragged(mb200_model* m, int32_t n_req, const int32_t* slots, const int64_t* prompt, const int32_t* prompt_off,
                                           const int64_t* neg_prompt, const uint8_t* vflags, const mb200_generate_params* params,
                                           int64_t* out_ids, int32_t out_ld, int32_t* out_len, void* stream) {
    MB_REQUIRE(m && m->finalized, "model not finalized");
    MB_REQUIRE(slots && prompt && prompt_off && vflags && params && out_ids && out_len, "null argument");
    const auto& c = m->cfg;
    cudaStream_t st = (cudaStream_t)stream;
    const bool use_cfg = neg_prompt != nullptr;
    const int N = n_req, rows = use_cfg ? 2 * N : N, nr = use_cfg ? 2 : 1;
    MB_REQUIRE(N >= 1 && rows <= m->max_rows, "requests exceed max_batch (rows double under classifier-free guidance)");
    MB_REQUIRE(prompt_off[0] == 0, "prompt offsets start at 0");
    const int d = c.d_model, V = c.vocab_size_out, ids_ld = c.tgt_seq_len, Vin = c.vocab_size_in;
    int n_splits_grid = 1, remaining = 0, first_poll = c.tgt_seq_len;
    for (int r = 0; r < N; ++r) {
        const mb200_generate_params& gp = params[r];
        const int P = prompt_off[r + 1] - prompt_off[r];
        MB_REQUIRE(P >= 1 && P < gp.max_length && gp.max_length <= c.tgt_seq_len, "need 1 <= prompt_len < max_length <= tgt_seq_len for every request");
        MB_REQUIRE(gp.max_length <= out_ld, "output rows are shorter than a request's max_length");
        MB_REQUIRE(slots[r] >= 0 && slots[r] < c.max_windows, "encoder slot out of range");
        MB_REQUIRE((gp.cfg_scale > 1.0f) == use_cfg, "classifier-free guidance on every request of a ragged call or on none");
        for (int t = prompt_off[r]; t < prompt_off[r + 1]; ++t) {
            MB_REQUIRE(prompt[t] >= 0 && prompt[t] < Vin, "prompt token id out of range");
            MB_REQUIRE(!use_cfg || (neg_prompt[t] >= 0 && neg_prompt[t] < Vin), "negative prompt token id out of range");
        }
        n_splits_grid = std::max(n_splits_grid, self_splits(gp.max_length));
        remaining = std::max(remaining, gp.max_length - (P + 1));
        first_poll = std::min(first_poll, std::min(std::max(gp.min_new_tokens, 1), gp.max_length - P));
    }

    const int total = prompt_off[N];
    std::vector<long long> pre((size_t)nr * total), idsrow((size_t)N * ids_ld, 0);
    std::vector<size_t> pre_off(N);
    std::vector<int> rowslot((size_t)3 * m->max_rows, 0);
    std::vector<unsigned char> state(sizeof(GenState) + (size_t)N * sizeof(RowState), 0);
    std::vector<SampleConfig> cfgs(N);
    reinterpret_cast<GenState*>(state.data())->n_req = N;
    RowState* rs = reinterpret_cast<RowState*>(state.data() + sizeof(GenState));
    size_t off = 0;
    for (int r = 0; r < N; ++r) {
        const mb200_generate_params& gp = params[r];
        const int P = prompt_off[r + 1] - prompt_off[r];
        pre_off[r] = off;
        for (int i = 0; i < nr; ++i) {
            const int64_t* src = (use_cfg && i == 0) ? neg_prompt : prompt;
            for (int t = 0; t < P; ++t) pre[off + (size_t)i * P + t] = src[prompt_off[r] + t];
        }
        off += (size_t)nr * P;
        for (int t = 0; t < P; ++t) idsrow[(size_t)r * ids_ld + t] = prompt[prompt_off[r] + t];
        for (int i = 0; i < nr; ++i) { rowslot[r + i * N] = slots[r]; rowslot[m->max_rows + 2 * r + i] = slots[r]; }
        rs[r].cur_len = P; rs[r].prompt_len = P; rs[r].max_length = gp.max_length; rs[r].min_new_tokens = gp.min_new_tokens;
        for (int t = 0; t < ids_ld; ++t) if (t >= P) idsrow[(size_t)r * ids_ld + t] = gp.pad_token_id;
        cfgs[r] = make_sample_config(&gp, N, use_cfg, V, ids_ld);
        cfgs[r].pos_rule_cumsum = 0; cfgs[r].vflags_ld = Vin;
    }
    MB_CUDA_CHECK(cudaMemcpyAsync(m->g_prefill_ids.p, pre.data(), pre.size() * 8, cudaMemcpyHostToDevice, st));
    MB_CUDA_CHECK(cudaMemcpyAsync(m->g_ids.p, idsrow.data(), idsrow.size() * 8, cudaMemcpyHostToDevice, st));
    MB_CUDA_CHECK(cudaMemsetAsync(m->g_keyvalid.p, 1, (size_t)m->max_rows * ids_ld, st));
    MB_CUDA_CHECK(cudaMemsetAsync(m->g_leftpad.p, 0, m->max_rows * sizeof(int), st));
    MB_CUDA_CHECK(cudaMemcpyAsync(m->g_rowslot.p, rowslot.data(), rowslot.size() * 4, cudaMemcpyHostToDevice, st));
    MB_CUDA_CHECK(cudaMemcpyAsync(m->g_vflags.p, vflags, (size_t)N * Vin, cudaMemcpyHostToDevice, st));
    MB_CUDA_CHECK(cudaMemcpyAsync(m->g_state.p, state.data(), state.size(), cudaMemcpyHostToDevice, st));
    MB_CUDA_CHECK(cudaMemcpyAsync(m->g_cfg.p, cfgs.data(), cfgs.size() * sizeof(SampleConfig), cudaMemcpyHostToDevice, st));
    MB_CUDA_CHECK(cudaMemsetAsync(m->d_ticket.p, 0, (size_t)m->max_rows * c.heads * sizeof(int), st));
    MB_CUDA_CHECK(cudaStreamSynchronize(st));

    GenState* gs = m->g_state.as<GenState>();
    MB_TRY(launch_prompt_scan_ragged(m->g_ids.as<long long>(), ids_ld, N, gs, m->g_vflags.as<unsigned char>(), Vin, cfgs[0].ts_start,
                                     cfgs[0].ts_end, m->g_lastts.as<int>(), st));
    for (int r = 0; r < N; ++r) {
        const int P = prompt_off[r + 1] - prompt_off[r];
        MB_TRY(decoder_prefill(m, nr, P, m->g_prefill_ids.as<long long>() + pre_off[r], 0, st, r, N, m->g_rowslot.as<int>() + m->max_rows + 2 * r));
        GemvParams g = final_logits_params(m, nr, m->p_x.as<float>() + (size_t)(P - 1) * d, (long long)P * d);
        g.seg[0].out += (size_t)r * V; g.seg[0].out_bs = (long long)N * V;
        MB_TRY(launch_gemv(g, st, false));
    }
    MB_TRY(launch_sample(sample_params(m, rows), N, st, false, true));

    auto key = std::make_tuple(rows, N, n_splits_grid, -1);
    auto it = m->graphs.find(key);
    if (it == m->graphs.end()) {
        cudaGraph_t graph;
        if (!m->cap_stream) MB_CUDA_CHECK(cudaStreamCreateWithFlags(&m->cap_stream, cudaStreamNonBlocking));
        MB_CUDA_CHECK(cudaStreamSynchronize(st));
        MB_CUDA_CHECK(cudaStreamBeginCapture(m->cap_stream, cudaStreamCaptureModeThreadLocal));
        const long long before = g_launch_count;
        int s = token_step(m, rows, N, n_splits_grid, m->cap_stream, m->use_pdl, nullptr, nullptr, true);
        cudaError_t e = cudaStreamEndCapture(m->cap_stream, &graph);
        m->graph_nodes[key] = g_launch_count - before;
        g_launch_count = before;
        if (s) return s;
        MB_CUDA_CHECK(e);
        cudaGraphExec_t exec;
        MB_CUDA_CHECK(cudaGraphInstantiate(&exec, graph, 0));
        cudaGraphDestroy(graph);
        it = m->graphs.emplace(key, exec).first;
    }
    int produced = 1;
    while (remaining > 0) {
        int burst = std::min(remaining, 16);
        if (first_poll > produced) burst = std::min(remaining, std::max(burst, first_poll - produced));
        for (int i = 0; i < burst; ++i) MB_CUDA_CHECK(cudaGraphLaunch(it->second, st));
        g_launch_count += (long long)burst * m->graph_nodes[key];
        remaining -= burst; produced += burst;
        MB_CUDA_CHECK(cudaMemcpyAsync(m->h_flag, &gs->all_finished, 4, cudaMemcpyDeviceToHost, st));
        MB_CUDA_CHECK(cudaStreamSynchronize(st));
        if (*m->h_flag) break;
    }
    MB_CUDA_CHECK(cudaMemcpyAsync(state.data(), m->g_state.p, state.size(), cudaMemcpyDeviceToHost, st));
    MB_CUDA_CHECK(cudaMemcpy2DAsync(out_ids, (size_t)out_ld * 8, m->g_ids.p, (size_t)ids_ld * 8, (size_t)std::min((int)out_ld, ids_ld) * 8, N,
                                    cudaMemcpyDeviceToHost, st));
    MB_CUDA_CHECK(cudaStreamSynchronize(st));
    for (int r = 0; r < N; ++r) {
        MB_REQUIRE(rs[r].finished && rs[r].cur_len <= params[r].max_length, "ragged token loop ended with an unfinished row");
        out_len[r] = rs[r].cur_len;
    }
    return 0;
}

static int ensure_beam_buffers(mb200_model* m) {
    const size_t R = (size_t)m->max_rows, ld = (size_t)m->cfg.tgt_seq_len, V = (size_t)m->cfg.vocab_size_out;
    MB_TRY(m->b_kvsrc.ensure(R * ld * sizeof(int)));
    MB_TRY(m->b_logprobs.ensure(R * V * sizeof(float)));
    MB_TRY(m->b_cand.ensure(R * V * sizeof(float)));
    MB_TRY(m->b_runscore.ensure(R * sizeof(float)));
    MB_TRY(m->b_finids[0].ensure(R * ld * 8)); MB_TRY(m->b_finids[1].ensure(R * ld * 8));
    MB_TRY(m->b_finscore.ensure(R * sizeof(float))); MB_TRY(m->b_finlen.ensure(R * sizeof(int)));
    MB_TRY(m->b_finflag.ensure(R)); MB_TRY(m->b_unsat.ensure(R));
    return 0;
}

static BeamParams beam_params(mb200_model* m, int rows, int K) {
    const int V = m->cfg.vocab_size_out;
    BeamParams bp{};
    bp.sample = sample_params(m, rows);
    bp.sample.logits = m->b_logprobs.as<float>(); bp.sample.logits_ld = V;
    bp.logits = m->d_logits.as<float>(); bp.logits_ld = V;
    bp.logprobs = m->b_logprobs.as<float>(); bp.cand = m->b_cand.as<float>(); bp.run_score = m->b_runscore.as<float>();
    bp.kv_src = m->b_kvsrc.as<int>(); bp.kv_src_ld = m->cfg.tgt_seq_len;
    bp.fin_ids[0] = m->b_finids[0].as<long long>(); bp.fin_ids[1] = m->b_finids[1].as<long long>();
    bp.fin_score = m->b_finscore.as<float>(); bp.fin_len = m->b_finlen.as<int>(); bp.fin_flag = m->b_finflag.as<unsigned char>();
    bp.unsat = m->b_unsat.as<unsigned char>();
    bp.K = K; bp.V = V; bp.ids_ld = m->cfg.tgt_seq_len;
    return bp;
}

extern "C" int mb200_model_generate_beams(mb200_model* m, const int32_t* slots, int32_t B, const int64_t* prompt, const uint8_t* prompt_mask,
                                          int32_t P, const int64_t* neg_prompt, const uint8_t* neg_mask, const uint8_t* vflags,
                                          const mb200_generate_params* gp, int32_t num_beams, int64_t fill_id, int64_t* out_ids,
                                          int32_t* out_len, float* out_scores, void* stream) {
    MB_REQUIRE(m && m->finalized, "model not finalized");
    MB_REQUIRE(slots && prompt && vflags && gp && out_ids && out_len && out_scores, "null argument");
    const auto& c = m->cfg;
    cudaStream_t st = (cudaStream_t)stream;
    const int K = num_beams;
    MB_REQUIRE(K >= 2 && K <= 4, "num_beams must be in [2, 4]");
    MB_REQUIRE(!gp->do_sample, "beam sampling (do_sample with num_beams > 1) is not supported");
    const bool use_cfg = neg_prompt != nullptr;
    const int BK = B * K, rows = use_cfg ? 2 * BK : BK;
    MB_REQUIRE(B >= 1 && rows <= m->max_rows, "batch * num_beams (x2 under classifier-free guidance) exceeds max_batch");
    MB_REQUIRE(P >= 1 && P < gp->max_length && gp->max_length <= c.tgt_seq_len, "need 1 <= prompt_len < max_length <= tgt_seq_len");
    for (int b = 0; b < B; ++b) MB_REQUIRE(slots[b] >= 0 && slots[b] < c.max_windows, "encoder slot out of range");
    const int d = c.d_model, V = c.vocab_size_out, ids_ld = c.tgt_seq_len;
    MB_REQUIRE(beam_select_smem_bytes(K, V, ids_ld) <= 220 * 1024, "beam candidates do not fit shared memory");
    MB_TRY(ensure_beam_buffers(m));

    std::vector<long long> pre((size_t)rows * P), idsrow((size_t)BK * ids_ld, (long long)gp->pad_token_id);
    std::vector<unsigned char> kv((size_t)rows * ids_ld, 1);
    std::vector<int> leftpad(rows, 0), rowslot(rows), kvsrc((size_t)rows * ids_ld, 0);
    for (int r = 0; r < rows; ++r) {
        const int b = (r % BK) / K;
        const bool neg_row = use_cfg && r < BK;
        const int64_t* src = neg_row ? neg_prompt : prompt;
        const uint8_t* msk = neg_row ? (neg_mask ? neg_mask : prompt_mask) : prompt_mask;
        int npad = 0; bool seen = false;
        for (int t = 0; t < P; ++t) {
            long long tok = src[(size_t)b * P + t];
            MB_REQUIRE(tok >= 0 && tok < c.vocab_size_in, "prompt token id out of range");
            pre[(size_t)r * P + t] = tok;
            unsigned char ok = msk ? (msk[(size_t)b * P + t] != 0) : 1;
            kv[(size_t)r * ids_ld + t] = ok;
            if (!ok && !seen) ++npad; else seen = true;
            kvsrc[(size_t)r * ids_ld + t] = r;
        }
        leftpad[r] = npad;
        rowslot[r] = slots[b];
    }
    for (int j = 0; j < BK; ++j)
        for (int t = 0; t < P; ++t) idsrow[(size_t)j * ids_ld + t] = prompt[(size_t)(j / K) * P + t];
    std::vector<float> runscore(BK), finscore(BK, -1.0e9f);
    for (int j = 0; j < BK; ++j) runscore[j] = j % K == 0 ? 0.f : -1.0e9f;
    GenState gs{};
    gs.cur_len = P; gs.prompt_len = P; gs.max_length = gp->max_length; gs.min_new_tokens = gp->min_new_tokens;
    const SampleConfig sc = make_sample_config(gp, BK, use_cfg, V, ids_ld);

    MB_CUDA_CHECK(cudaMemcpyAsync(m->g_prefill_ids.p, pre.data(), pre.size() * 8, cudaMemcpyHostToDevice, st));
    MB_CUDA_CHECK(cudaMemcpyAsync(m->g_ids.p, idsrow.data(), idsrow.size() * 8, cudaMemcpyHostToDevice, st));
    MB_CUDA_CHECK(cudaMemcpyAsync(m->g_keyvalid.p, kv.data(), kv.size(), cudaMemcpyHostToDevice, st));
    MB_CUDA_CHECK(cudaMemcpyAsync(m->g_leftpad.p, leftpad.data(), rows * 4, cudaMemcpyHostToDevice, st));
    MB_CUDA_CHECK(cudaMemcpyAsync(m->g_rowslot.p, rowslot.data(), rows * 4, cudaMemcpyHostToDevice, st));
    MB_CUDA_CHECK(cudaMemcpyAsync(m->g_vflags.p, vflags, c.vocab_size_in, cudaMemcpyHostToDevice, st));
    MB_CUDA_CHECK(cudaMemcpyAsync(m->g_state.p, &gs, sizeof(gs), cudaMemcpyHostToDevice, st));
    MB_CUDA_CHECK(cudaMemcpyAsync(m->g_cfg.p, &sc, sizeof(sc), cudaMemcpyHostToDevice, st));
    MB_CUDA_CHECK(cudaMemcpyAsync(m->b_kvsrc.p, kvsrc.data(), kvsrc.size() * 4, cudaMemcpyHostToDevice, st));
    MB_CUDA_CHECK(cudaMemcpyAsync(m->b_runscore.p, runscore.data(), BK * 4, cudaMemcpyHostToDevice, st));
    MB_CUDA_CHECK(cudaMemcpyAsync(m->b_finscore.p, finscore.data(), BK * 4, cudaMemcpyHostToDevice, st));
    MB_CUDA_CHECK(cudaMemsetAsync(m->b_finlen.p, 0, BK * sizeof(int), st));
    MB_CUDA_CHECK(cudaMemsetAsync(m->b_finflag.p, 0, BK, st));
    MB_CUDA_CHECK(cudaMemsetAsync(m->b_unsat.p, 1, B, st));
    MB_CUDA_CHECK(cudaMemsetAsync(m->d_ticket.p, 0, (size_t)m->max_rows * m->cfg.heads * sizeof(int), st));
    MB_CUDA_CHECK(cudaStreamSynchronize(st));

    const BeamParams bp = beam_params(m, rows, K);

    MB_TRY(launch_prompt_scan(m->g_ids.as<long long>(), ids_ld, BK, P, m->g_vflags.as<unsigned char>(), sc.ts_start, sc.ts_end,
                              m->g_lastts.as<int>(), st));
    MB_TRY(decoder_prefill(m, rows, P, m->g_prefill_ids.as<long long>(), gp->position_rule, st));
    MB_TRY(final_logits(m, rows, m->p_x.as<float>() + (size_t)(P - 1) * d, (long long)P * d, st, false));
    MB_TRY(launch_beam_step(bp, B, st));

    const int n_splits_self = self_splits(gp->max_length);
    auto key = std::make_tuple(rows, (int)B, n_splits_self, K);
    auto it = m->graphs.find(key);
    if (it == m->graphs.end()) {
        cudaGraph_t graph;
        if (!m->cap_stream) MB_CUDA_CHECK(cudaStreamCreateWithFlags(&m->cap_stream, cudaStreamNonBlocking));
        MB_CUDA_CHECK(cudaStreamSynchronize(st));
        MB_CUDA_CHECK(cudaStreamBeginCapture(m->cap_stream, cudaStreamCaptureModeThreadLocal));
        const long long before = g_launch_count;
        int s = token_step(m, rows, B, n_splits_self, m->cap_stream, m->use_pdl, nullptr, &bp);
        cudaError_t e = cudaStreamEndCapture(m->cap_stream, &graph);
        m->graph_nodes[key] = g_launch_count - before;
        g_launch_count = before;
        if (s) return s;
        MB_CUDA_CHECK(e);
        cudaGraphExec_t exec;
        MB_CUDA_CHECK(cudaGraphInstantiate(&exec, graph, 0));
        cudaGraphDestroy(graph);
        it = m->graphs.emplace(key, exec).first;
    }
    int remaining = gp->max_length - (P + 1);
    MB_CUDA_CHECK(cudaMemcpyAsync(m->h_flag, &m->g_state.as<GenState>()->all_finished, 4, cudaMemcpyDeviceToHost, st));
    MB_CUDA_CHECK(cudaStreamSynchronize(st));
    if (*m->h_flag) remaining = 0;
    while (remaining > 0) {
        const int burst = std::min(remaining, 16);
        for (int i = 0; i < burst; ++i) MB_CUDA_CHECK(cudaGraphLaunch(it->second, st));
        g_launch_count += (long long)burst * m->graph_nodes[key];
        remaining -= burst;
        MB_CUDA_CHECK(cudaMemcpyAsync(m->h_flag, &m->g_state.as<GenState>()->all_finished, 4, cudaMemcpyDeviceToHost, st));
        MB_CUDA_CHECK(cudaStreamSynchronize(st));
        if (*m->h_flag) break;
    }
    GenState fin{};
    MB_CUDA_CHECK(cudaMemcpyAsync(&fin, m->g_state.p, sizeof(fin), cudaMemcpyDeviceToHost, st));
    MB_CUDA_CHECK(cudaStreamSynchronize(st));
    std::vector<long long> fids((size_t)BK * ids_ld);
    std::vector<int> flen(BK);
    std::vector<unsigned char> fflag(BK);
    MB_CUDA_CHECK(cudaMemcpyAsync(fids.data(), m->b_finids[fin.step & 1].p, fids.size() * 8, cudaMemcpyDeviceToHost, st));
    MB_CUDA_CHECK(cudaMemcpyAsync(finscore.data(), m->b_finscore.p, BK * 4, cudaMemcpyDeviceToHost, st));
    MB_CUDA_CHECK(cudaMemcpyAsync(flen.data(), m->b_finlen.p, BK * 4, cudaMemcpyDeviceToHost, st));
    MB_CUDA_CHECK(cudaMemcpyAsync(fflag.data(), m->b_finflag.p, BK, cudaMemcpyDeviceToHost, st));
    MB_CUDA_CHECK(cudaStreamSynchronize(st));
    int gen_max = 0;
    for (int b = 0; b < B; ++b) {
        MB_REQUIRE(fflag[(size_t)b * K], "beam search ended without a finished hypothesis");
        gen_max = std::max(gen_max, flen[(size_t)b * K]);
    }
    const int Lout = P + gen_max;
    for (int b = 0; b < B; ++b) {
        const long long* h = fids.data() + (size_t)b * K * ids_ld;
        const int Lb = P + flen[(size_t)b * K];
        for (int t = 0; t < Lout; ++t) out_ids[(size_t)b * Lout + t] = t < Lb ? h[t] : fill_id;
        out_scores[b] = finscore[(size_t)b * K];
    }
    *out_len = Lout;
    return 0;
}

extern "C" int mb200_model_forward_logits(mb200_model* m, const int32_t* slots, int32_t B, const int64_t* ids, const uint8_t* mask,
                                          int32_t len, int32_t position_rule, float* logits_out, void* stream) {
    MB_REQUIRE(m && m->finalized, "model not finalized");
    MB_REQUIRE(B >= 1 && B <= m->max_rows && len >= 1 && len <= m->cfg.tgt_seq_len, "bad batch / length");
    const auto& c = m->cfg;
    cudaStream_t st = (cudaStream_t)stream;
    const int ids_ld = c.tgt_seq_len, d = c.d_model;
    std::vector<unsigned char> kv((size_t)B * ids_ld, 1);
    std::vector<int> leftpad(B, 0), rowslot(B);
    std::vector<long long> pre((size_t)B * len);
    for (int b = 0; b < B; ++b) {
        int npad = 0; bool seen = false;
        for (int t = 0; t < len; ++t) {
            long long tok = ids[(size_t)b * len + t];
            MB_REQUIRE(tok >= 0 && tok < c.vocab_size_in, "token id out of range");
            pre[(size_t)b * len + t] = tok;
            unsigned char ok = mask ? (mask[(size_t)b * len + t] != 0) : 1;
            kv[(size_t)b * ids_ld + t] = ok;
            if (!ok && !seen) ++npad; else seen = true;
        }
        leftpad[b] = npad; rowslot[b] = slots[b];
    }
    MB_CUDA_CHECK(cudaMemcpyAsync(m->g_prefill_ids.p, pre.data(), pre.size() * 8, cudaMemcpyHostToDevice, st));
    MB_CUDA_CHECK(cudaMemcpyAsync(m->g_keyvalid.p, kv.data(), kv.size(), cudaMemcpyHostToDevice, st));
    MB_CUDA_CHECK(cudaMemcpyAsync(m->g_leftpad.p, leftpad.data(), B * 4, cudaMemcpyHostToDevice, st));
    MB_CUDA_CHECK(cudaMemcpyAsync(m->g_rowslot.p, rowslot.data(), B * 4, cudaMemcpyHostToDevice, st));
    MB_CUDA_CHECK(cudaStreamSynchronize(st));
    MB_TRY(decoder_prefill(m, B, len, m->g_prefill_ids.as<long long>(), position_rule, st));
    const int R = B * len;
    MB_TRY(layernorm(m->p_x.as<float>(), m->p_h.as<float>(), m->dec_ln_w, m->dec_ln_b, R, d, 1e-5f, st));
    MB_TRY(launch_gemm(gemm_base(plain_map(m->p_h.as<float>(), d), m->proj_out, d, plain_map(logits_out, c.vocab_size_out), nullptr, R,
                                 c.vocab_size_out, d), st, &m->gemm));
    return 0;
}

extern "C" int mb200_model_set_option(mb200_model* m, const char* name, int value) {
    MB_REQUIRE(m && name, "null argument");
    if (!strcmp(name, "pdl")) {
        if (m->use_pdl != (value != 0)) {
            for (auto& g : m->graphs) cudaGraphExecDestroy(g.second);
            m->graphs.clear();
        }
        m->use_pdl = value != 0;
        return 0;
    }
    if (!strcmp(name, "mega")) { m->use_mega = value; return 0; }
    if (!strcmp(name, "ll_sleep")) return mega2_set_poll_sleep(value);
    if (!strcmp(name, "enc_graph")) { m->enc_graph = value; return 0; }
    if (!strcmp(name, "trace_cta")) { m->trace_cta = value; return 0; }
    if (!strcmp(name, "ll_debug")) return mega2_set_debug(value);
    if (!strcmp(name, "ll_reps")) {
        MB_REQUIRE(value >= 1 && value <= MEGA_LL_MAX_REPS && value * 2 <= 32, "ll_reps must be in [1, 16]");
        m->ll.reps = value;
        return 0;
    }
    if (!strcmp(name, "mega_trace")) {
        if (value) { MB_TRY(m->mega_trace.ensure(128 * 16 * 8)); MB_CUDA_CHECK(cudaMemset(m->mega_trace.p, 0, 128 * 16 * 8)); }
        return 0;
    }
    set_last_error(std::string("unknown option ") + name);
    return 2;
}

extern "C" int mb200_model_profile_step(mb200_model* m, int32_t rows, int32_t B, int32_t max_length, int32_t iters, float* out_us, void* stream) {
    MB_REQUIRE(m && m->finalized && out_us && iters >= 1, "bad argument");
    cudaStream_t st = (cudaStream_t)stream;
    MB_CUDA_CHECK(cudaStreamSynchronize(st));
    GenState gs{};
    MB_CUDA_CHECK(cudaMemcpy(&gs, m->g_state.p, sizeof(gs), cudaMemcpyDeviceToHost));
    const int cur0 = gs.prompt_len + 1;
    double acc[3] = {0, 0, 0}; long long cnt[3] = {0, 0, 0};
    if (!g_prof.created) { for (auto& e : g_prof.ev) MB_CUDA_CHECK(cudaEventCreate(&e)); g_prof.created = true; }
    const int n_splits_self = self_splits(max_length);
    for (int it = 0; it < iters; ++it) {
        gs.cur_len = cur0 + it; gs.all_finished = 0; gs.n_finished = 0; gs.ticket = 0; gs.max_length = m->cfg.tgt_seq_len; gs.min_new_tokens = 0;
        MB_CUDA_CHECK(cudaMemcpy(m->g_state.p, &gs, sizeof(gs), cudaMemcpyHostToDevice));
        MB_CUDA_CHECK(cudaMemset(m->g_finished.p, 0, m->max_rows));
        g_prof.n = 0; g_prof.on = true;
        int s = token_step(m, rows, B, n_splits_self, st, false);
        g_prof.on = false;
        if (s) return s;
        MB_CUDA_CHECK(cudaStreamSynchronize(st));
        for (int i = 0; i < g_prof.n; ++i) {
            float ms = 0.f;
            MB_CUDA_CHECK(cudaEventElapsedTime(&ms, g_prof.ev[2 * i], g_prof.ev[2 * i + 1]));
            acc[g_prof.cls[i]] += ms * 1000.0; cnt[g_prof.cls[i]]++;
        }
    }
    for (int c = 0; c < 3; ++c) out_us[c] = (float)(acc[c] / iters);
    out_us[3] = (float)((cnt[0] / iters) * 1000000LL + (cnt[1] / iters) * 1000LL + (cnt[2] / iters));
    return 0;
}

extern "C" int mb200_model_read_trace(mb200_model* m, uint64_t* out, int32_t n_phases) {
    MB_REQUIRE(m && out && m->mega_trace.p && n_phases <= 128, "trace not enabled");
    MB_CUDA_CHECK(cudaDeviceSynchronize());
    MB_CUDA_CHECK(cudaMemcpy(out, m->mega_trace.p, (size_t)n_phases * 16 * 8, cudaMemcpyDeviceToHost));
    return 0;
}

extern "C" int mb200_model_mega_stats(mb200_model* m, double* out, int32_t reset) {
    MB_REQUIRE(m && out, "null argument");
    out[0] = (double)m->mega_launches; out[1] = m->mega_ms; out[2] = (double)m->mega_tokens;
    if (reset) { m->mega_launches = 0; m->mega_ms = 0.0; m->mega_tokens = 0; }
    return 0;
}

extern "C" int mb200_model_logits_chain(mb200_model* m, const float* logits, int32_t B, int32_t use_cfg, const int64_t* ids, int32_t L,
                                        int32_t prompt_len, const uint8_t* vflags, const mb200_generate_params* gp, int32_t step,
                                        int32_t has_last_scores, float* scores_out, int64_t* chosen_out, void* stream) {
    MB_REQUIRE(m && m->finalized && logits && ids && vflags && gp && scores_out && chosen_out, "null argument");
    const auto& c = m->cfg;
    const int rows = use_cfg ? 2 * B : B, V = c.vocab_size_out, ids_ld = c.tgt_seq_len;
    MB_REQUIRE(B >= 1 && rows <= m->max_rows && L >= 1 && L < ids_ld, "bad batch / length");
    cudaStream_t st = (cudaStream_t)stream;
    std::vector<long long> idsrow((size_t)B * ids_ld, (long long)gp->pad_token_id);
    for (int b = 0; b < B; ++b)
        for (int t = 0; t < L; ++t) idsrow[(size_t)b * ids_ld + t] = ids[(size_t)b * L + t];
    GenState gs{};
    gs.cur_len = L; gs.prompt_len = prompt_len; gs.max_length = gp->max_length; gs.min_new_tokens = gp->min_new_tokens;
    gs.step = step; gs.has_last_scores = has_last_scores;
    const SampleConfig sc = make_sample_config(gp, B, use_cfg != 0, V, ids_ld);
    std::vector<int> zeros(rows, 0);
    MB_CUDA_CHECK(cudaMemcpyAsync(m->g_ids.p, idsrow.data(), idsrow.size() * 8, cudaMemcpyHostToDevice, st));
    MB_CUDA_CHECK(cudaMemcpyAsync(m->g_vflags.p, vflags, c.vocab_size_in, cudaMemcpyHostToDevice, st));
    MB_CUDA_CHECK(cudaMemcpyAsync(m->g_state.p, &gs, sizeof(gs), cudaMemcpyHostToDevice, st));
    MB_CUDA_CHECK(cudaMemcpyAsync(m->g_cfg.p, &sc, sizeof(sc), cudaMemcpyHostToDevice, st));
    MB_CUDA_CHECK(cudaMemcpyAsync(m->g_leftpad.p, zeros.data(), rows * 4, cudaMemcpyHostToDevice, st));
    MB_CUDA_CHECK(cudaMemsetAsync(m->g_finished.p, 0, m->max_rows, st));
    MB_CUDA_CHECK(cudaMemcpyAsync(m->d_logits.p, logits, (size_t)rows * V * 4, cudaMemcpyDeviceToDevice, st));
    MB_CUDA_CHECK(cudaStreamSynchronize(st));
    MB_TRY(launch_prompt_scan(m->g_ids.as<long long>(), ids_ld, B, L, m->g_vflags.as<unsigned char>(), sc.ts_start, sc.ts_end, m->g_lastts.as<int>(), st));
    SampleParams sp = sample_params(m, rows);
    sp.dbg_scores = scores_out;
    MB_TRY(launch_sample(sp, B, st, false));
    std::vector<long long> chosen(B);
    MB_CUDA_CHECK(cudaMemcpy2DAsync(chosen.data(), 8, m->g_ids.as<long long>() + L, (size_t)ids_ld * 8, 8, B, cudaMemcpyDeviceToHost, st));
    MB_CUDA_CHECK(cudaStreamSynchronize(st));
    for (int b = 0; b < B; ++b) chosen_out[b] = chosen[b];
    return 0;
}

extern "C" int mb200_model_beam_step(mb200_model* m, const float* logits, int32_t B, int32_t num_beams, int32_t use_cfg, const int64_t* ids,
                                     int32_t L, int32_t prompt_len, const uint8_t* vflags, const mb200_generate_params* gp,
                                     const float* run_scores, int32_t step, int32_t has_last_scores, float* logprobs_out, int32_t* top_out,
                                     int32_t* parent_out, int64_t* token_out, float* score_out, float* fin_score_out, int32_t* fin_len_out,
                                     uint8_t* fin_flag_out, int64_t* fin_ids_out, void* stream) {
    MB_REQUIRE(m && m->finalized && logits && ids && vflags && gp && run_scores && logprobs_out && top_out && parent_out && token_out &&
               score_out && fin_score_out && fin_len_out && fin_flag_out && fin_ids_out, "null argument");
    const auto& c = m->cfg;
    const int K = num_beams, BK = B * K, rows = use_cfg ? 2 * BK : BK, V = c.vocab_size_out, ids_ld = c.tgt_seq_len;
    MB_REQUIRE(K >= 2 && K <= 4, "num_beams must be in [2, 4]");
    MB_REQUIRE(B >= 1 && rows <= m->max_rows && prompt_len >= 1 && L >= prompt_len && L < ids_ld && L < gp->max_length, "bad batch / length");
    MB_REQUIRE(beam_select_smem_bytes(K, V, ids_ld) <= 220 * 1024, "beam candidates do not fit shared memory");
    cudaStream_t st = (cudaStream_t)stream;
    MB_TRY(ensure_beam_buffers(m));
    std::vector<long long> idsrow((size_t)BK * ids_ld, (long long)gp->pad_token_id);
    for (int j = 0; j < BK; ++j)
        for (int t = 0; t < L; ++t) idsrow[(size_t)j * ids_ld + t] = ids[(size_t)j * L + t];
    GenState gs{};
    gs.cur_len = L; gs.prompt_len = prompt_len; gs.max_length = gp->max_length; gs.min_new_tokens = gp->min_new_tokens;
    gs.step = step; gs.has_last_scores = has_last_scores;
    const SampleConfig sc = make_sample_config(gp, BK, use_cfg != 0, V, ids_ld);
    std::vector<int> zeros(rows, 0);
    std::vector<float> empty(BK, -1.0e9f);
    MB_CUDA_CHECK(cudaMemcpyAsync(m->g_ids.p, idsrow.data(), idsrow.size() * 8, cudaMemcpyHostToDevice, st));
    MB_CUDA_CHECK(cudaMemcpyAsync(m->g_vflags.p, vflags, c.vocab_size_in, cudaMemcpyHostToDevice, st));
    MB_CUDA_CHECK(cudaMemcpyAsync(m->g_state.p, &gs, sizeof(gs), cudaMemcpyHostToDevice, st));
    MB_CUDA_CHECK(cudaMemcpyAsync(m->g_cfg.p, &sc, sizeof(sc), cudaMemcpyHostToDevice, st));
    MB_CUDA_CHECK(cudaMemcpyAsync(m->g_leftpad.p, zeros.data(), rows * 4, cudaMemcpyHostToDevice, st));
    MB_CUDA_CHECK(cudaMemsetAsync(m->b_kvsrc.p, 0, (size_t)rows * ids_ld * sizeof(int), st));
    MB_CUDA_CHECK(cudaMemcpyAsync(m->b_runscore.p, run_scores, BK * 4, cudaMemcpyHostToDevice, st));
    MB_CUDA_CHECK(cudaMemcpyAsync(m->b_finscore.p, empty.data(), BK * 4, cudaMemcpyHostToDevice, st));
    MB_CUDA_CHECK(cudaMemsetAsync(m->b_finlen.p, 0, BK * sizeof(int), st));
    MB_CUDA_CHECK(cudaMemsetAsync(m->b_finflag.p, 0, BK, st));
    MB_CUDA_CHECK(cudaMemsetAsync(m->b_unsat.p, 1, B, st));
    MB_CUDA_CHECK(cudaMemcpyAsync(m->d_logits.p, logits, (size_t)rows * V * 4, cudaMemcpyDeviceToDevice, st));
    MB_CUDA_CHECK(cudaStreamSynchronize(st));
    MB_TRY(launch_prompt_scan(m->g_ids.as<long long>(), ids_ld, BK, L, m->g_vflags.as<unsigned char>(), sc.ts_start, sc.ts_end,
                              m->g_lastts.as<int>(), st));
    BeamParams bp = beam_params(m, rows, K);
    bp.dbg_logprobs = logprobs_out;
    MB_TRY(m->b_dbg.ensure((size_t)2 * m->max_rows * sizeof(int)));
    bp.dbg_top = m->b_dbg.as<int>(); bp.dbg_parent = m->b_dbg.as<int>() + m->max_rows;
    MB_TRY(launch_beam_step(bp, B, st));
    std::vector<int> dbg((size_t)2 * m->max_rows);
    std::vector<long long> tok((size_t)BK * ids_ld), fids((size_t)BK * ids_ld);
    MB_CUDA_CHECK(cudaMemcpyAsync(dbg.data(), m->b_dbg.p, dbg.size() * 4, cudaMemcpyDeviceToHost, st));
    MB_CUDA_CHECK(cudaMemcpyAsync(tok.data(), m->g_ids.p, tok.size() * 8, cudaMemcpyDeviceToHost, st));
    MB_CUDA_CHECK(cudaMemcpyAsync(fids.data(), m->b_finids[1 - (step & 1)].p, fids.size() * 8, cudaMemcpyDeviceToHost, st));
    MB_CUDA_CHECK(cudaMemcpyAsync(score_out, m->b_runscore.p, BK * 4, cudaMemcpyDeviceToHost, st));
    MB_CUDA_CHECK(cudaMemcpyAsync(fin_score_out, m->b_finscore.p, BK * 4, cudaMemcpyDeviceToHost, st));
    MB_CUDA_CHECK(cudaMemcpyAsync(fin_len_out, m->b_finlen.p, BK * 4, cudaMemcpyDeviceToHost, st));
    MB_CUDA_CHECK(cudaMemcpyAsync(fin_flag_out, m->b_finflag.p, BK, cudaMemcpyDeviceToHost, st));
    MB_CUDA_CHECK(cudaStreamSynchronize(st));
    for (int j = 0; j < BK; ++j) {
        top_out[j] = dbg[j]; parent_out[j] = dbg[m->max_rows + j]; token_out[j] = tok[(size_t)j * ids_ld + L];
        for (int t = 0; t <= L; ++t) fin_ids_out[(size_t)j * (L + 1) + t] = fids[(size_t)j * ids_ld + t];
    }
    return 0;
}
```

mapperatorinator_b200/csrc/gemm.cu:

```cuda
#include <algorithm>
#include <cstdlib>
#include "common.cuh"
#include "kernels.h"

namespace mb200 {

namespace {

constexpr int BM = 128, BN = 128, BK = 16, PAD = 4;

__global__ void __launch_bounds__(256, 2) gemm_f32_kernel(GemmParams p) {
    __shared__ __align__(16) float As[2][BK][BM + PAD];
    __shared__ __align__(16) float Bs[2][BK][BN + PAD];

    const int tid = threadIdx.x;
    const int tx = tid & 15, ty = tid >> 4;
    const long long m0 = (long long)blockIdx.y * BM;
    const int n0 = blockIdx.x * BN;

    const int lrow = tid >> 2;
    const int lk = (tid & 3) * 4;
    const float* a_ptr[2];
    const float* w_ptr[2];
    bool a_ok[2], w_ok[2];
#pragma unroll
    for (int h = 0; h < 2; ++h) {
        long long m = m0 + lrow + h * 64;
        a_ok[h] = m < p.M;
        a_ptr[h] = a_ok[h] ? p.A.row(p.m_base + m) : p.A.ptr;
        int n = n0 + lrow + h * 64;
        w_ok[h] = n < p.N;
        w_ptr[h] = p.W + (long long)(w_ok[h] ? n : 0) * p.ldw;
    }

    float acc[8][8];
#pragma unroll
    for (int i = 0; i < 8; ++i)
#pragma unroll
        for (int j = 0; j < 8; ++j) acc[i][j] = 0.f;

    float4 ra[2], rw[2];
    const int k_lo_ = p.splitk > 1 ? blockIdx.z * p.k_per_split : 0;
    const int k_hi_ = p.splitk > 1 ? min(p.K, k_lo_ + p.k_per_split) : p.K;
    auto gload = [&](int k0) {
#pragma unroll
        for (int h = 0; h < 2; ++h) {
            int k = k_lo_ + k0 + lk;
            ra[h] = (a_ok[h] && k < k_hi_) ? __ldg(reinterpret_cast<const float4*>(a_ptr[h] + k)) : make_float4(0, 0, 0, 0);
            rw[h] = (w_ok[h] && k < k_hi_) ? __ldg(reinterpret_cast<const float4*>(w_ptr[h] + k)) : make_float4(0, 0, 0, 0);
        }
    };
    auto sstore = [&](int buf) {
#pragma unroll
        for (int h = 0; h < 2; ++h) {
            int r = lrow + h * 64;
            As[buf][lk + 0][r] = ra[h].x; As[buf][lk + 1][r] = ra[h].y; As[buf][lk + 2][r] = ra[h].z; As[buf][lk + 3][r] = ra[h].w;
            Bs[buf][lk + 0][r] = rw[h].x; Bs[buf][lk + 1][r] = rw[h].y; Bs[buf][lk + 2][r] = rw[h].z; Bs[buf][lk + 3][r] = rw[h].w;
        }
    };

    const int k_lo = p.splitk > 1 ? blockIdx.z * p.k_per_split : 0;
    const int k_hi = p.splitk > 1 ? min(p.K, k_lo + p.k_per_split) : p.K;
    const int nk = (k_hi - k_lo + BK - 1) / BK;
    gload(0);
    sstore(0);
    __syncthreads();
    for (int kt = 0; kt < nk; ++kt) {
        const int buf = kt & 1;
        if (kt + 1 < nk) gload((kt + 1) * BK);
#pragma unroll
        for (int k = 0; k < BK; ++k) {
            float4 a0 = *reinterpret_cast<const float4*>(&As[buf][k][ty * 4]);
            float4 a1 = *reinterpret_cast<const float4*>(&As[buf][k][64 + ty * 4]);
            float4 b0 = *reinterpret_cast<const float4*>(&Bs[buf][k][tx * 4]);
            float4 b1 = *reinterpret_cast<const float4*>(&Bs[buf][k][64 + tx * 4]);
            float a[8] = {a0.x, a0.y, a0.z, a0.w, a1.x, a1.y, a1.z, a1.w};
            float b[8] = {b0.x, b0.y, b0.z, b0.w, b1.x, b1.y, b1.z, b1.w};
#pragma unroll
            for (int i = 0; i < 8; ++i)
#pragma unroll
                for (int j = 0; j < 8; ++j) acc[i][j] = fmaf(a[i], b[j], acc[i][j]);
        }
        if (kt + 1 < nk) {
            sstore(buf ^ 1);
            __syncthreads();
        }
    }

    if (p.splitk > 1) {
#pragma unroll
        for (int i = 0; i < 8; ++i) {
            long long m = m0 + (i < 4 ? ty * 4 + i : 64 + ty * 4 + (i - 4));
            if (m >= p.M) continue;
            float* wrow = p.splitk_ws + ((long long)blockIdx.z * p.M + m) * p.N;
#pragma unroll
            for (int jh = 0; jh < 2; ++jh)
#pragma unroll
                for (int j = 0; j < 4; ++j) {
                    int nn = n0 + jh * 64 + tx * 4 + j;
                    if (nn < p.N) wrow[nn] = acc[i][jh * 4 + j];
                }
        }
        return;
    }
#pragma unroll
    for (int i = 0; i < 8; ++i) {
        long long m = m0 + (i < 4 ? ty * 4 + i : 64 + ty * 4 + (i - 4));
        if (m >= p.M) continue;
        float* crow = p.C.row(p.m_base + m);
        const float* rrow = p.R.ptr ? p.R.row(p.m_base + m) : nullptr;
        const float* grow = p.gate ? p.gate + ((p.m_base + m) / p.gate_rpb) * p.gate_ld : nullptr;
#pragma unroll
        for (int jh = 0; jh < 2; ++jh) {
            int n = n0 + jh * 64 + tx * 4;
#pragma unroll
            for (int j = 0; j < 4; ++j) {
                int nn = n + j;
                if (nn >= p.N) continue;
                float v = acc[i][jh * 4 + j];
                if (p.bias) v += __ldg(p.bias + nn);
                v = apply_act(v, p.act) * p.alpha;
                if (grow) v *= __ldg(grow + nn);
                if (rrow) v += rrow[nn];
                crow[nn] = v;
            }
        }
    }
}

__global__ void __launch_bounds__(256) gemm_splitk_reduce_kernel(GemmParams p) {
    const long long idx = (long long)blockIdx.x * 256 + threadIdx.x;
    if (idx >= (long long)p.M * p.N) return;
    const long long m = idx / p.N;
    const int n = (int)(idx - m * p.N);
    float v = p.splitk_ws[m * p.N + n];
    for (int z = 1; z < p.splitk; ++z) v += p.splitk_ws[((long long)z * p.M + m) * p.N + n];
    if (p.bias) v += __ldg(p.bias + n);
    v = apply_act(v, p.act) * p.alpha;
    if (p.gate) v *= __ldg(p.gate + ((p.m_base + m) / p.gate_rpb) * p.gate_ld + n);
    if (p.R.ptr) v += p.R.row(p.m_base + m)[n];
    p.C.row(p.m_base + m)[n] = v;
}

}

int GemmCtx::reserve(size_t splitk_need, size_t a_split_need) {
    auto grow = [&](float*& ptr, size_t& have, size_t need) -> int {
        if (need <= have) return 0;
        MB_REQUIRE(!frozen, "GEMM scratch is referenced by a captured CUDA graph and cannot grow (reserve the largest shape before capturing)");
        if (ptr) MB_CUDA_CHECK(cudaFree(ptr));
        ptr = nullptr; have = 0;
        MB_CUDA_CHECK(cudaMalloc(&ptr, need));
        have = need;
        return 0;
    };
    int s = grow(splitk_ws, splitk_bytes, splitk_need);
    if (s) return s;
    s = grow(a_split, a_split_bytes, a_split_need);
    if (s) return s;
    if (!tc_err) { MB_CUDA_CHECK(cudaMalloc(&tc_err, 4)); MB_CUDA_CHECK(cudaMemset(tc_err, 0, 4)); }
    return 0;
}

int GemmCtx::error() {
    if (!tc_err) return 0;
    int h = 0;
    cudaMemcpy(&h, tc_err, 4, cudaMemcpyDeviceToHost);
    return h;
}

void GemmCtx::destroy() {
    for (auto& kv : mirrors) cudaFree(const_cast<float*>(kv.second.hi));
    mirrors.clear();
    if (splitk_ws) cudaFree(splitk_ws);
    if (a_split) cudaFree(a_split);
    if (tc_err) cudaFree(tc_err);
    splitk_ws = a_split = nullptr; tc_err = nullptr; splitk_bytes = a_split_bytes = 0; frozen = false;
}

GemmCtx* default_gemm_ctx() {
    static GemmCtx ctx;
    static bool init = false;
    if (!init) {
        int dev = 0;
        cudaGetDevice(&dev);
        cudaDeviceGetAttribute(&ctx.num_sms, cudaDevAttrMultiProcessorCount, dev);
        init = true;
    }
    return &ctx;
}

int gemm_splits_simt(int N, int K, int num_sms, int* k_per_split) {
    const int tiles_n = (N + BN - 1) / BN;
    int splits = 1;
    if (tiles_n * 2 <= num_sms && K >= 64) splits = std::max(1, std::min((num_sms + tiles_n - 1) / tiles_n, K / 32));
    const int kps = ((K + splits - 1) / splits + BK - 1) / BK * BK;
    splits = (K + kps - 1) / kps;
    *k_per_split = kps;
    return splits;
}

int launch_splitk_reduce(const GemmParams& q, cudaStream_t stream) {
    gemm_splitk_reduce_kernel<<<(unsigned)(((long long)q.M * q.N + 255) / 256), 256, 0, stream>>>(q);
    MB_LAUNCH_CHECK();
    ++g_launch_count;
    return 0;
}

int launch_gemm(const GemmParams& p, cudaStream_t stream, GemmCtx* ctx) {
    MB_REQUIRE(ctx != nullptr, "GEMM needs its engine's scratch context");
    MB_REQUIRE(p.K % 4 == 0, "GEMM K must be a multiple of 4 (float4 loads)");
    MB_REQUIRE(p.A.ld % 4 == 0 && p.ldw % 4 == 0, "GEMM operand row strides must be multiples of 4 floats");
    MB_REQUIRE((reinterpret_cast<uintptr_t>(p.A.ptr) & 15) == 0 && (reinterpret_cast<uintptr_t>(p.W) & 15) == 0,
               "GEMM operands must be 16-byte aligned");
    if (p.M <= 0 || p.N <= 0) return 0;
    if (tc_gemm_eligible(p, ctx)) return launch_gemm_tc(p, stream, ctx);
    int kps = 0;
    const int splits = gemm_splits_simt(p.N, p.K, ctx->num_sms, &kps);
    const int tiles_n = (p.N + BN - 1) / BN;
    if (splits == 1) {
        dim3 grid(tiles_n, (unsigned)((p.M + BM - 1) / BM));
        gemm_f32_kernel<<<grid, 256, 0, stream>>>(p);
        MB_LAUNCH_CHECK();
        ++g_launch_count;
        return 0;
    }
    const size_t row_bytes = (size_t)splits * p.N * sizeof(float);
    if (row_bytes * (size_t)p.M > ctx->splitk_bytes && !ctx->frozen) {
        const int s = ctx->reserve(std::max(row_bytes * (size_t)std::min(p.M, 2048), (size_t)64 << 20), 0);
        if (s) return s;
    }
    MB_REQUIRE(ctx->splitk_bytes >= row_bytes * BM, "split-K workspace smaller than one row tile");
    const long long rows_per_pass = std::min<long long>(p.M, (long long)(ctx->splitk_bytes / row_bytes) / BM * BM);
    for (long long m0 = 0; m0 < p.M; m0 += rows_per_pass) {
        GemmParams q = p;
        q.m_base = p.m_base + m0;
        q.M = (int)std::min<long long>(rows_per_pass, p.M - m0);
        q.splitk_ws = ctx->splitk_ws; q.splitk = splits; q.k_per_split = kps; q.split_mode = 1;
        gemm_f32_kernel<<<dim3(tiles_n, (unsigned)((q.M + BM - 1) / BM), splits), 256, 0, stream>>>(q);
        MB_LAUNCH_CHECK();
        ++g_launch_count;
        const int s = launch_splitk_reduce(q, stream);
        if (s) return s;
    }
    return 0;
}

}
```

mapperatorinator_b200/engine.py:

```python
from __future__ import annotations

import ctypes as C
from typing import Dict, List, Optional, Sequence

import numpy as np
import torch

from . import _lib
from .config import DiTConfig, MelConfig, ModelConfig
from .filterbank import mel_filterbank
from .token_layout import TokenLayout

VF_EOS, VF_TIMED, VF_SOS, VF_LB_EOS, VF_BEAT, VF_MANIA, VF_SCROLL = 1, 2, 4, 8, 16, 32, 64


def _stream() -> int:
    return torch.cuda.current_stream().cuda_stream


def _mel_c(cfg: MelConfig) -> _lib.MelConfigC:
    return _lib.MelConfigC(cfg.n_fft, cfg.hop_length, cfg.n_mels, 1 if cfg.pad_mode == "reflect" else 0, 1 if cfg.log_scale else 0)


class MelEngine:

    def __init__(self, cfg: MelConfig, mel_basis: Optional[np.ndarray] = None):
        self.cfg = cfg
        self.lib = _lib.load()
        basis = np.ascontiguousarray(mel_filterbank(cfg) if mel_basis is None else mel_basis, dtype=np.float32)
        assert basis.shape == (cfg.n_mels, cfg.n_fft // 2 + 1)
        self.handle = C.c_void_p()
        cc = _mel_c(cfg)
        _lib.check(self.lib.mb200_mel_create(C.byref(self.handle), C.byref(cc), basis.ctypes.data))

    def forward(self, samples: torch.Tensor) -> torch.Tensor:
        assert samples.is_cuda and samples.dtype == torch.float32 and samples.dim() == 2
        samples = samples.contiguous()
        B, n = samples.shape
        out = torch.empty(B, n // self.cfg.hop_length + 1, self.cfg.n_mels, device=samples.device, dtype=torch.float32)
        _lib.check(self.lib.mb200_mel_forward(self.handle, samples.data_ptr(), B, n, out.data_ptr(), _stream()))
        return out

    def __del__(self):
        try:
            if getattr(self, "handle", None):
                self.lib.mb200_mel_destroy(self.handle)
        except Exception:
            pass


def build_vflags(layout: TokenLayout, eos_ids: Sequence[int]) -> np.ndarray:
    f = np.zeros(layout.vocab_size_in, dtype=np.uint8)
    for ids, bit in ((eos_ids, VF_EOS), (layout.timed_token_ids(), VF_TIMED), (layout.sos_ids(), VF_SOS),
                     (layout.lookback_eos_ids(), VF_LB_EOS), (layout.beat_type_tokens(), VF_BEAT),
                     (layout.mania_type_tokens(), VF_MANIA), (layout.scroll_speed_tokens(), VF_SCROLL)):
        if len(ids):
            f[np.asarray(list(ids), dtype=np.int64)] |= bit
    return f


class ModelEngine:

    def __init__(self, cfg: ModelConfig, state_dict: Dict[str, torch.Tensor], max_windows: int = 32, max_batch: int = 16,
                 mel_basis: Optional[np.ndarray] = None, device: str = "cuda:0"):
        if not torch.cuda.is_available():
            raise RuntimeError("mapperatorinator_b200 needs a CUDA device (sm_90a); there is no CPU path")
        self.cfg = cfg
        self.device = torch.device(device)
        self.lib = _lib.load()
        self.max_windows, self.max_batch = max_windows, max_batch
        basis = np.ascontiguousarray(mel_filterbank(cfg.mel) if mel_basis is None else mel_basis, dtype=np.float32)
        cc = _lib.ModelConfigC(cfg.d_model, cfg.encoder_layers, cfg.decoder_layers, cfg.heads, cfg.ffn_dim, cfg.src_seq_len,
                               cfg.tgt_seq_len, cfg.vocab_size_in, cfg.vocab_size_out, _mel_c(cfg.mel), max_windows, max_batch)
        self.handle = C.c_void_p()
        with torch.cuda.device(self.device):
            _lib.check(self.lib.mb200_model_create(C.byref(self.handle), C.byref(cc), basis.ctypes.data))
            for name, t in state_dict.items():
                if not isinstance(t, torch.Tensor) or not t.is_floating_point():
                    continue
                a = t.detach().to("cpu", torch.float32).contiguous().numpy()
                _lib.check(self.lib.mb200_model_set_weight(self.handle, name.encode(), a.ctypes.data, a.size))
            _lib.check(self.lib.mb200_model_finalize(self.handle))

    def encode(self, pcm: torch.Tensor, slot_begin: int = 0, return_states: bool = False) -> Optional[torch.Tensor]:
        assert pcm.is_cuda and pcm.dtype == torch.float32 and pcm.dim() == 2 and pcm.shape[1] == self.cfg.samples_per_window
        pcm = pcm.contiguous()
        n = pcm.shape[0]
        out = None
        if return_states:
            out = torch.empty(n, self.cfg.max_source_positions, self.cfg.d_model, device=pcm.device, dtype=torch.float32)
        with torch.cuda.device(self.device):
            _lib.check(self.lib.mb200_model_encode(self.handle, pcm.data_ptr(), n, slot_begin, out.data_ptr() if out is not None else None,
                                                   _stream()))
        return out

    def _generate_params(self, layout: TokenLayout, generate_kwargs: dict, position_rule: str = "arange"):
        gk = dict(generate_kwargs)
        t = float(gk.get("temperature", 1.0))
        types_first = bool(gk.get("types_first", False))
        lookback_time = float(gk.get("lookback_time", 0.0))
        lookahead_time = float(gk.get("lookahead_time", 0.0))
        ctx = gk.get("context_type")
        eos_ids = layout.eos_token_ids(lookback_time, lookahead_time, ctx)
        p = _lib.GenerateParamsC()
        p.cfg_scale = float(gk.get("cfg_scale", 1.0))
        p.timeshift_bias = float(gk.get("timeshift_bias", 0))
        p.types_first = int(types_first)
        p.temperature = t
        p.timing_temperature = float(gk.get("timing_temperature", t))
        p.mania_column_temperature = float(gk.get("mania_column_temperature", t))
        p.taiko_hit_temperature = float(gk.get("taiko_hit_temperature", t))
        conds = []
        if types_first:
            if p.timing_temperature != t and layout.beat_type_tokens():
                conds.append((p.timing_temperature, 1, VF_BEAT))
            if p.mania_column_temperature != t and layout.mania_type_tokens():
                conds.append((p.mania_column_temperature, 3, VF_MANIA))
            if p.taiko_hit_temperature != t and layout.scroll_speed_tokens():
                conds.append((p.taiko_hit_temperature, 1, VF_SCROLL))
        p.n_cond = len(conds)
        for i, (ct, off, fl) in enumerate(conds):
            p.cond_temp[i], p.cond_offset[i], p.cond_flag[i] = ct, off, fl
        p.lookback_on = int(lookback_time > 0)
        p.lookback_start = layout.time_shift_start
        p.lookback_end = layout.lookback_end(lookback_time) if lookback_time > 0 else layout.time_shift_start
        p.do_sample = int(bool(gk.get("do_sample", False)))
        p.top_k = int(gk.get("top_k", 0) or 0)
        p.top_p = float(gk.get("top_p", 1.0) if gk.get("top_p") is not None else 1.0)
        p.top_p_cut = 1.0 - float(gk.get("top_p", 1.0) if gk.get("top_p") is not None else 1.0)
        p.max_length = int(gk.get("max_length", self.cfg.tgt_seq_len))
        p.min_new_tokens = int(gk.get("min_new_tokens") or 0)
        pad = gk.get("pad_token_id", layout.pad_id)
        p.pad_token_id = int(layout.pad_id if pad is None else pad)
        seed = gk.get("seed")
        if seed is None:
            seed = int(torch.randint(0, 2 ** 62, (1,)).item()) if p.do_sample else 0
        p.seed = int(seed) & 0xFFFFFFFFFFFFFFFF
        p.time_shift_start, p.time_shift_end = layout.time_shift_start, layout.time_shift_end
        p.position_rule = {"arange": 0, "mask_cumsum": 1}[position_rule]
        return p, eos_ids, gk

    def generate(self, slots: Sequence[int], prompt: torch.Tensor, prompt_mask: Optional[torch.Tensor], layout: TokenLayout,
                 generate_kwargs: dict, negative_prompt: Optional[torch.Tensor] = None,
                 negative_mask: Optional[torch.Tensor] = None, position_rule: str = "arange") -> torch.Tensor:
        if int(generate_kwargs.get("num_beams", 1) or 1) != 1:
            return self.generate_beams(slots, prompt, prompt_mask, layout, generate_kwargs, negative_prompt, negative_mask,
                                       position_rule)[0]
        p, eos_ids, gk = self._generate_params(layout, generate_kwargs, position_rule)
        B, P = prompt.shape
        use_cfg = negative_prompt is not None and p.cfg_scale > 1.0

        ids = np.ascontiguousarray(prompt.detach().cpu().numpy().astype(np.int64))
        msk = None if prompt_mask is None else np.ascontiguousarray(prompt_mask.detach().cpu().numpy().astype(np.uint8))
        neg = nmsk = None
        if use_cfg:
            neg_full = ids.copy()
            npn = negative_prompt.detach().cpu().numpy().astype(np.int64)
            neg_full[:, :npn.shape[1]] = npn
            neg = np.ascontiguousarray(neg_full)
            nmsk = np.ascontiguousarray(msk.copy() if msk is not None else np.ones_like(ids, dtype=np.uint8))
        vflags = build_vflags(layout, eos_ids)
        slots_a = np.ascontiguousarray(np.asarray(list(slots), dtype=np.int32))
        assert slots_a.shape[0] == B
        out = np.zeros((B, p.max_length), dtype=np.int64)
        out_len = C.c_int32(0)
        with torch.cuda.device(self.device):
            _lib.check(self.lib.mb200_model_generate(
                self.handle, slots_a.ctypes.data, B, ids.ctypes.data, None if msk is None else msk.ctypes.data, P,
                None if neg is None else neg.ctypes.data, None if nmsk is None else nmsk.ctypes.data, vflags.ctypes.data,
                C.byref(p), out.ctypes.data, C.byref(out_len), _stream()))
        L = out_len.value
        return torch.from_numpy(out.reshape(-1)[: B * L].reshape(B, L).copy())

    def generate_ragged(self, requests: Sequence[tuple], layout: TokenLayout) -> List[torch.Tensor]:
        n = len(requests)
        if n == 0:
            return []
        params = (_lib.GenerateParamsC * n)()
        vflags = np.zeros((n, layout.vocab_size_in), dtype=np.uint8)
        prompts, negs, cfg_rows = [], [], []
        for r, (slot, prompt, gk, neg) in enumerate(requests):
            if int(gk.get("num_beams", 1) or 1) != 1:
                raise ValueError("a ragged call takes greedy or sampling requests; beam search (num_beams > 1) goes through generate()")
            p, eos_ids, _ = self._generate_params(layout, gk)
            ids = np.asarray(torch.as_tensor(prompt).detach().cpu().numpy(), dtype=np.int64).reshape(-1)
            if not 1 <= ids.shape[0] < p.max_length <= self.cfg.tgt_seq_len:
                raise ValueError(f"request {r}: need 1 <= prompt length ({ids.shape[0]}) < max_length ({p.max_length}) <= "
                                 f"{self.cfg.tgt_seq_len}")
            use_cfg = neg is not None and p.cfg_scale > 1.0
            cfg_rows.append(use_cfg)
            if not use_cfg:
                p.cfg_scale = 1.0
            neg_full = ids.copy()
            if use_cfg:
                npn = np.asarray(torch.as_tensor(neg).detach().cpu().numpy(), dtype=np.int64).reshape(-1)
                neg_full[:npn.shape[0]] = npn
            params[r] = p
            vflags[r] = build_vflags(layout, eos_ids)
            prompts.append(ids); negs.append(neg_full)
        if any(cfg_rows) and not all(cfg_rows):
            raise ValueError("classifier-free guidance (negative prompt and cfg_scale > 1) on every request of a ragged call or on none")
        rows = n * (2 if cfg_rows[0] else 1)
        if rows > self.max_batch:
            raise ValueError(f"{n} requests{' x 2 (classifier-free guidance)' if cfg_rows[0] else ''} = {rows} decoder rows; this engine "
                             f"was built with max_batch={self.max_batch}")
        off = np.zeros(n + 1, dtype=np.int32)
        off[1:] = np.cumsum([len(x) for x in prompts])
        flat = np.ascontiguousarray(np.concatenate(prompts))
        nflat = np.ascontiguousarray(np.concatenate(negs)) if cfg_rows[0] else None
        slots_a = np.ascontiguousarray(np.asarray([int(q[0]) for q in requests], dtype=np.int32))
        ld = max(int(params[r].max_length) for r in range(n))
        out = np.zeros((n, ld), dtype=np.int64)
        out_len = np.zeros(n, dtype=np.int32)
        with torch.cuda.device(self.device):
            _lib.check(self.lib.mb200_model_generate_ragged(
                self.handle, n, slots_a.ctypes.data, flat.ctypes.data, off.ctypes.data, None if nflat is None else nflat.ctypes.data,
                vflags.ctypes.data, C.cast(params, C.c_void_p), out.ctypes.data, ld, out_len.ctypes.data, _stream()))
        return [torch.from_numpy(out[r, :out_len[r]].copy())[None] for r in range(n)]

    def generate_beams(self, slots: Sequence[int], prompt: torch.Tensor, prompt_mask: Optional[torch.Tensor], layout: TokenLayout,
                       generate_kwargs: dict, negative_prompt: Optional[torch.Tensor] = None,
                       negative_mask: Optional[torch.Tensor] = None, position_rule: str = "arange"):
        gk = dict(generate_kwargs)
        K = int(gk.get("num_beams", 1) or 1)
        if not 2 <= K <= 4:
            raise ValueError(f"num_beams={K}: beam search takes 2..4 beams (the candidates of one item live in one CTA's shared memory)")
        if gk.get("do_sample", False):
            raise ValueError("do_sample with num_beams > 1 (beam sampling) is not supported")
        if int(gk.get("num_return_sequences", 1) or 1) != 1:
            raise ValueError("num_return_sequences != 1 is not supported")
        if gk.get("length_penalty") not in (None, 1.0) or gk.get("early_stopping") not in (None, False):
            raise ValueError("beam search supports only the default length_penalty (1.0) and early_stopping (False)")
        p, eos_ids, gk = self._generate_params(layout, gk, position_rule)
        B, P = prompt.shape
        use_cfg = negative_prompt is not None and p.cfg_scale > 1.0
        rows = B * K * (2 if use_cfg else 1)
        if rows > self.max_batch:
            raise ValueError(f"beam search needs batch * num_beams{' * 2 (classifier-free guidance)' if use_cfg else ''} = {rows} "
                             f"decoder rows; this engine was built with max_batch={self.max_batch}")
        ids = np.ascontiguousarray(prompt.detach().cpu().numpy().astype(np.int64))
        msk = None if prompt_mask is None else np.ascontiguousarray(prompt_mask.detach().cpu().numpy().astype(np.uint8))
        neg = nmsk = None
        if use_cfg:
            neg_full = ids.copy()
            npn = negative_prompt.detach().cpu().numpy().astype(np.int64)
            neg_full[:, :npn.shape[1]] = npn
            neg = np.ascontiguousarray(neg_full)
            nmsk = np.ascontiguousarray(msk.copy() if msk is not None else np.ones_like(ids, dtype=np.uint8))
        vflags = build_vflags(layout, eos_ids)
        slots_a = np.ascontiguousarray(np.asarray(list(slots), dtype=np.int32))
        assert slots_a.shape[0] == B
        fill = p.pad_token_id if p.pad_token_id else eos_ids[0]
        out = np.zeros((B, p.max_length), dtype=np.int64)
        scores = np.zeros(B, dtype=np.float32)
        out_len = C.c_int32(0)
        with torch.cuda.device(self.device):
            _lib.check(self.lib.mb200_model_generate_beams(
                self.handle, slots_a.ctypes.data, B, ids.ctypes.data, None if msk is None else msk.ctypes.data, P,
                None if neg is None else neg.ctypes.data, None if nmsk is None else nmsk.ctypes.data, vflags.ctypes.data,
                C.byref(p), K, int(fill), out.ctypes.data, C.byref(out_len), scores.ctypes.data, _stream()))
        L = out_len.value
        return torch.from_numpy(out.reshape(-1)[: B * L].reshape(B, L).copy()), torch.from_numpy(scores)

    def logits_chain(self, logits: torch.Tensor, ids: torch.Tensor, prompt_len: int, layout: TokenLayout, generate_kwargs: dict,
                     step: int = 0, has_last_scores: bool = False, use_cfg: bool = False):
        p, eos_ids, gk = self._generate_params(layout, generate_kwargs)
        B, L = ids.shape
        a = np.ascontiguousarray(ids.detach().cpu().numpy().astype(np.int64))
        vflags = build_vflags(layout, eos_ids)
        logits = logits.contiguous().float()
        scores = torch.empty(B, self.cfg.vocab_size_out, device=logits.device, dtype=torch.float32)
        chosen = np.zeros(B, dtype=np.int64)
        with torch.cuda.device(self.device):
            _lib.check(self.lib.mb200_model_logits_chain(self.handle, logits.data_ptr(), B, int(use_cfg), a.ctypes.data, L, int(prompt_len),
                                                         vflags.ctypes.data, C.byref(p), int(step), int(has_last_scores), scores.data_ptr(),
                                                         chosen.ctypes.data, _stream()))
        return scores, torch.from_numpy(chosen)

    def beam_step(self, logits: torch.Tensor, ids: torch.Tensor, run_scores: torch.Tensor, num_beams: int, prompt_len: int,
                  layout: TokenLayout, generate_kwargs: dict, step: int = 0, has_last_scores: bool = False, use_cfg: bool = False) -> dict:
        p, eos_ids, gk = self._generate_params(layout, generate_kwargs)
        BK, L = ids.shape
        B = BK // num_beams
        a = np.ascontiguousarray(ids.detach().cpu().numpy().astype(np.int64))
        rs = np.ascontiguousarray(run_scores.detach().cpu().numpy().astype(np.float32))
        vflags = build_vflags(layout, eos_ids)
        logits = logits.contiguous().float()
        lp = torch.empty(BK, self.cfg.vocab_size_out, device=logits.device, dtype=torch.float32)
        out = dict(top=np.zeros(BK, np.int32), parent=np.zeros(BK, np.int32), token=np.zeros(BK, np.int64), score=np.zeros(BK, np.float32),
                   fin_score=np.zeros(BK, np.float32), fin_len=np.zeros(BK, np.int32), fin_flag=np.zeros(BK, np.uint8),
                   fin_ids=np.zeros((BK, L + 1), np.int64))
        with torch.cuda.device(self.device):
            _lib.check(self.lib.mb200_model_beam_step(
                self.handle, logits.data_ptr(), B, int(num_beams), int(use_cfg), a.ctypes.data, L, int(prompt_len), vflags.ctypes.data,
                C.byref(p), rs.ctypes.data, int(step), int(has_last_scores), lp.data_ptr(), out["top"].ctypes.data,
                out["parent"].ctypes.data, out["token"].ctypes.data, out["score"].ctypes.data, out["fin_score"].ctypes.data,
                out["fin_len"].ctypes.data, out["fin_flag"].ctypes.data, out["fin_ids"].ctypes.data, _stream()))
        res = {k: torch.from_numpy(v) for k, v in out.items()}
        res["logprobs"] = lp.cpu()
        return res

    def forward_logits(self, slots: Sequence[int], ids: torch.Tensor, mask: Optional[torch.Tensor],
                       position_rule: str = "arange") -> torch.Tensor:
        B, L = ids.shape
        a = np.ascontiguousarray(ids.detach().cpu().numpy().astype(np.int64))
        m = None if mask is None else np.ascontiguousarray(mask.detach().cpu().numpy().astype(np.uint8))
        slots_a = np.ascontiguousarray(np.asarray(list(slots), dtype=np.int32))
        out = torch.empty(B, L, self.cfg.vocab_size_out, device=self.device, dtype=torch.float32)
        with torch.cuda.device(self.device):
            _lib.check(self.lib.mb200_model_forward_logits(self.handle, slots_a.ctypes.data, B, a.ctypes.data,
                                                           None if m is None else m.ctypes.data, L,
                                                           {"arange": 0, "mask_cumsum": 1}[position_rule], out.data_ptr(), _stream()))
        return out

    def set_option(self, name: str, value: int) -> None:
        _lib.check(self.lib.mb200_model_set_option(self.handle, name.encode(), int(value)))

    def __del__(self):
        try:
            if getattr(self, "handle", None):
                self.lib.mb200_model_destroy(self.handle)
        except Exception:
            pass


class DiTEngine:

    def __init__(self, cfg: DiTConfig, state_dict: Dict[str, torch.Tensor], max_seq_len: int = 1024, max_batch: int = 2,
                 device: str = "cuda:0"):
        if not torch.cuda.is_available():
            raise RuntimeError("mapperatorinator_b200 needs a CUDA device (sm_90a); there is no CPU path")
        self.cfg = cfg
        self.device = torch.device(device)
        self.lib = _lib.load()
        cc = _lib.DitConfigC(cfg.hidden, cfg.depth, cfg.heads, cfg.mlp_ratio, cfg.in_channels, cfg.context_size, cfg.class_size,
                             cfg.pos_freq_dim, cfg.t_freq_dim, max_seq_len, max_batch)
        self.handle = C.c_void_p()
        with torch.cuda.device(self.device):
            _lib.check(self.lib.mb200_dit_create(C.byref(self.handle), C.byref(cc)))
            for name, t in state_dict.items():
                a = t.detach().to("cpu", torch.float32).contiguous().numpy()
                _lib.check(self.lib.mb200_dit_set_weight(self.handle, name.encode(), a.ctypes.data, a.size))
            _lib.check(self.lib.mb200_dit_finalize(self.handle))
        self._mask_keep = None

    def _mask(self, mask_mode: str, band: int, dense: Optional[torch.Tensor]) -> _lib.DitMaskC:
        mm = {"none": 0, "band": 2, "dense": 3}[mask_mode]
        self._mask_keep = dense
        return _lib.DitMaskC(mm, int(band), None if dense is None else dense.data_ptr())

    def forward_with_cfg(self, x, t, c, y, cfg_scale: float, mask_mode: str = "none", band: int = 0, dense=None) -> torch.Tensor:
        N, _, T = x.shape
        x, c, y = x.contiguous().float(), c.contiguous().float(), y.contiguous().float()
        tt = np.ascontiguousarray(t.detach().cpu().numpy().astype(np.int32))
        out = torch.empty(N, self.cfg.out_channels, T, device=x.device, dtype=torch.float32)
        mk = self._mask(mask_mode, band, dense)
        with torch.cuda.device(self.device):
            _lib.check(self.lib.mb200_dit_forward_with_cfg(self.handle, x.data_ptr(), tt.ctypes.data, c.data_ptr(), y.data_ptr(), N, T,
                                                           float(cfg_scale), C.byref(mk), out.data_ptr(), _stream()))
        return out

    def sample_loop(self, z, c, y, cfg_scale: float, schedule_rows: np.ndarray, noise: torch.Tensor,
                    inpaint: Optional[torch.Tensor] = None, mask_mode: str = "none", band: int = 0, dense=None) -> torch.Tensor:
        N, _, T = z.shape
        z, c, y, noise = z.contiguous().float(), c.contiguous().float(), y.contiguous().float(), noise.contiguous().float()
        sched = np.ascontiguousarray(schedule_rows, dtype=np.float32)
        steps = sched.shape[0]
        assert noise.shape == (steps, N, 2, T)
        ip = None if inpaint is None else inpaint.to(torch.uint8).contiguous()
        out = torch.empty_like(z)
        mk = self._mask(mask_mode, band, dense)
        with torch.cuda.device(self.device):
            _lib.check(self.lib.mb200_dit_sample_loop(self.handle, z.data_ptr(), c.data_ptr(), y.data_ptr(),
                                                      None if ip is None else ip.data_ptr(), N, T, float(cfg_scale), C.byref(mk),
                                                      sched.ctypes.data, steps, noise.data_ptr(), out.data_ptr(), _stream()))
        return out

    CURVE_TYPES = {"Bezier": 0, "PerfectCurve": 1, "Catmull": 2, "Linear": 3, None: 0}

    def set_sliders(self, sliders) -> int:
        sl = list(sliders or [])
        if not sl:
            _lib.check(self.lib.mb200_dit_set_sliders(self.handle, 0, None, None, None, None, None))
            return 0
        off = np.zeros(len(sl) + 1, dtype=np.int32)
        off[1:] = np.cumsum([len(s[1]) for s in sl])
        idx = np.ascontiguousarray(np.concatenate([np.asarray(s[1], dtype=np.int32) for s in sl]))
        end = np.ascontiguousarray([int(s[2]) for s in sl], dtype=np.int32)
        typ = np.ascontiguousarray([self.CURVE_TYPES.get(s[0], 0) for s in sl], dtype=np.int32)
        length = np.ascontiguousarray([float(s[3]) for s in sl], dtype=np.float32)
        with torch.cuda.device(self.device):
            _lib.check(self.lib.mb200_dit_set_sliders(self.handle, len(sl), off.ctypes.data, idx.ctypes.data, end.ctypes.data, typ.ctypes.data,
                                                      length.ctypes.data))
        return len(sl)

    def apply_sliders(self, x: torch.Tensor) -> torch.Tensor:
        x = x.contiguous().float().clone()
        with torch.cuda.device(self.device):
            _lib.check(self.lib.mb200_dit_apply_sliders(self.handle, x.data_ptr(), x.shape[0], x.shape[2], _stream()))
        return x

    def __del__(self):
        try:
            if getattr(self, "handle", None):
                self.lib.mb200_dit_destroy(self.handle)
        except Exception:
            pass
```

Measured before the change: 1811.

## Add small-grid attention/GEMM variants, pinned staging, and cached vocab flags

Templates the fallback attention kernel so grids with fewer blocks than SMs use one query row per thread-row plus a register prefetch of the next K/V tile. The SIMT GEMM gets a half-height M tile when M is small, which raises block count. Generation inputs are staged through a pinned host buffer guarded by an event, which removes a stream sync. Output ids are read back through that buffer before the megakernel's existing sync, which removes two extra syncs. Python caches vocab flag arrays per layout. Together these target low occupancy on small problems and per-call host overhead, at the cost of more template instantiations and a staging buffer whose size must cover the inputs.

Result: faster. 1869 (median of 6 runs) (+3.2%).

```diff
diff --git a/mapperatorinator_b200/csrc/attention.cu b/mapperatorinator_b200/csrc/attention.cu
--- a/mapperatorinator_b200/csrc/attention.cu
+++ b/mapperatorinator_b200/csrc/attention.cu
@@ -17,7 +17,9 @@
     }
 }
 
+template <int QPT>
 __global__ void __launch_bounds__(256) attention_kernel(AttentionParams p) {
+    constexpr int TQ_ = 16 * QPT;
     extern __shared__ __align__(16) float smem[];
     float (*Qt)[LDS_] = reinterpret_cast<float (*)[LDS_]>(smem);
     float (*Kt)[LDS_] = reinterpret_cast<float (*)[LDS_]>(smem + HD * LDS_);
@@ -25,7 +27,7 @@
     float (*Ps)[LDS_] = reinterpret_cast<float (*)[LDS_]>(smem + 3 * HD * LDS_);
 
     const int tid = threadIdx.x, tx = tid & 15, ty = tid >> 4;
-    const int q0 = blockIdx.x * TQ, h = blockIdx.y, b = blockIdx.z;
+    const int q0 = blockIdx.x * TQ_, h = blockIdx.y, b = blockIdx.z;
     const float* qb = p.q + (long long)b * p.q_bs + h * HD;
     const int kvb = p.kv_slot ? p.kv_slot[b] : b;
     const float* kb = p.k + (long long)kvb * p.k_bs + h * HD;
@@ -34,7 +36,7 @@
     {
         const int r = tid >> 4, dq = (tid & 15) * 4;
 #pragma unroll
-        for (int rr = 0; rr < 4; ++rr) {
+        for (int rr = 0; rr < QPT; ++rr) {
             int row = r + rr * 16, q = q0 + row;
             float4 v = q < p.Tq ? *reinterpret_cast<const float4*>(qb + (long long)q * p.q_ld + dq) : make_float4(0, 0, 0, 0);
             Qt[dq + 0][row] = v.x * p.scale; Qt[dq + 1][row] = v.y * p.scale;
@@ -44,60 +46,79 @@
 
     int kt_begin = 0, kt_end = (p.Tk + TK - 1) / TK;
     if (p.mask_mode == MASK_CAUSAL) {
-        int last = p.q_pos0 + min(q0 + TQ - 1, p.Tq - 1);
+        int last = p.q_pos0 + min(q0 + TQ_ - 1, p.Tq - 1);
         kt_end = min(kt_end, last / TK + 1);
     } else if (p.mask_mode == MASK_BAND) {
-        int lo = q0 - p.band + 1, hi = min(q0 + TQ - 1, p.Tq - 1) + p.band;
+        int lo = q0 - p.band + 1, hi = min(q0 + TQ_ - 1, p.Tq - 1) + p.band;
         kt_begin = max(0, lo) / TK;
         kt_end = min(kt_end, hi / TK + 1);
     }
 
-    float m_i[4], l_i[4], o[4][4];
-#pragma unroll
-    for (int i = 0; i < 4; ++i) {
+    float m_i[QPT], l_i[QPT], o[QPT][4];
+#pragma unroll
+    for (int i = 0; i < QPT; ++i) {
         m_i[i] = -INFINITY; l_i[i] = 0.f;
 #pragma unroll
         for (int j = 0; j < 4; ++j) o[i][j] = 0.f;
     }
+
+    constexpr bool AHEAD = QPT == 1;
+    float4 kr[4], vr[4];
+    auto gload = [&](int k0) {
+        const int r = tid >> 4, dq = (tid & 15) * 4;
+#pragma unroll
+        for (int rr = 0; rr < 4; ++rr) {
+            int k = k0 + r + rr * 16;
+            kr[rr] = make_float4(0, 0, 0, 0); vr[rr] = make_float4(0, 0, 0, 0);
+            if (k < p.Tk) {
+                kr[rr] = *reinterpret_cast<const float4*>(kb + (long long)k * p.k_ld + dq);
+                vr[rr] = *reinterpret_cast<const float4*>(vb + (long long)k * p.v_ld + dq);
+            }
+        }
+    };
+    if (AHEAD && kt_begin < kt_end) gload(kt_begin * TK);
 
     for (int kt = kt_begin; kt < kt_end; ++kt) {
         const int k0 = kt * TK;
         __syncthreads();
+        if (!AHEAD) gload(k0);
         {
             const int r = tid >> 4, dq = (tid & 15) * 4;
 #pragma unroll
             for (int rr = 0; rr < 4; ++rr) {
-                int row = r + rr * 16, k = k0 + row;
-                float4 kv = make_float4(0, 0, 0, 0), vv = make_float4(0, 0, 0, 0);
-                if (k < p.Tk) {
-                    kv = *reinterpret_cast<const float4*>(kb + (long long)k * p.k_ld + dq);
-                    vv = *reinterpret_cast<const float4*>(vb + (long long)k * p.v_ld + dq);
-                }
-                Kt[dq + 0][row] = kv.x; Kt[dq + 1][row] = kv.y; Kt[dq + 2][row] = kv.z; Kt[dq + 3][row] = kv.w;
-                *reinterpret_cast<float4*>(&Vs[row][dq]) = vv;
+                int row = r + rr * 16;
+                Kt[dq + 0][row] = kr[rr].x; Kt[dq + 1][row] = kr[rr].y; Kt[dq + 2][row] = kr[rr].z; Kt[dq + 3][row] = kr[rr].w;
+                *reinterpret_cast<float4*>(&Vs[row][dq]) = vr[rr];
             }
         }
         __syncthreads();
-
-        float s[4][4];
-#pragma unroll
-        for (int i = 0; i < 4; ++i)
+        if (AHEAD && kt + 1 < kt_end) gload(k0 + TK);
+
+        float s[QPT][4];
+#pragma unroll
+        for (int i = 0; i < QPT; ++i)
 #pragma unroll
             for (int j = 0; j < 4; ++j) s[i][j] = 0.f;
 #pragma unroll 16
         for (int d = 0; d < HD; ++d) {
-            float4 qa = *reinterpret_cast<const float4*>(&Qt[d][ty * 4]);
+            float qv[QPT];
+            if constexpr (QPT == 4) {
+                float4 qa = *reinterpret_cast<const float4*>(&Qt[d][ty * 4]);
+                qv[0] = qa.x; qv[1] = qa.y; qv[2] = qa.z; qv[3] = qa.w;
+            } else {
+                qv[0] = Qt[d][ty];
+            }
             float4 ka = *reinterpret_cast<const float4*>(&Kt[d][tx * 4]);
-            float qv[4] = {qa.x, qa.y, qa.z, qa.w}, kv[4] = {ka.x, ka.y, ka.z, ka.w};
-#pragma unroll
-            for (int i = 0; i < 4; ++i)
+            float kv[4] = {ka.x, ka.y, ka.z, ka.w};
+#pragma unroll
+            for (int i = 0; i < QPT; ++i)
 #pragma unroll
                 for (int j = 0; j < 4; ++j) s[i][j] = fmaf(qv[i], kv[j], s[i][j]);
         }
 
 #pragma unroll
-        for (int i = 0; i < 4; ++i) {
-            const int q = q0 + ty * 4 + i;
+        for (int i = 0; i < QPT; ++i) {
+            const int q = q0 + ty * QPT + i;
             float mx = -INFINITY;
 #pragma unroll
             for (int j = 0; j < 4; ++j) {
@@ -115,23 +136,23 @@
                 pr[j] = (s[i][j] == -INFINITY) ? 0.f : expf(s[i][j] - m_new);
                 psum += pr[j];
             }
-            l_i[i] = l_i[i] * corr + psum;
+            l_i[i] = fmaf(l_i[i], corr, psum);
             m_i[i] = m_new;
 #pragma unroll
             for (int j = 0; j < 4; ++j) o[i][j] *= corr;
-            *reinterpret_cast<float4*>(&Ps[ty * 4 + i][tx * 4]) = make_float4(pr[0], pr[1], pr[2], pr[3]);
+            *reinterpret_cast<float4*>(&Ps[ty * QPT + i][tx * 4]) = make_float4(pr[0], pr[1], pr[2], pr[3]);
         }
         __syncthreads();
 
 #pragma unroll 4
         for (int c4 = 0; c4 < TK / 4; ++c4) {
-            float4 pa[4], va[4];
-#pragma unroll
-            for (int i = 0; i < 4; ++i) pa[i] = *reinterpret_cast<const float4*>(&Ps[ty * 4 + i][c4 * 4]);
+            float4 pa[QPT], va[4];
+#pragma unroll
+            for (int i = 0; i < QPT; ++i) pa[i] = *reinterpret_cast<const float4*>(&Ps[ty * QPT + i][c4 * 4]);
 #pragma unroll
             for (int c = 0; c < 4; ++c) va[c] = *reinterpret_cast<const float4*>(&Vs[c4 * 4 + c][tx * 4]);
 #pragma unroll
-            for (int i = 0; i < 4; ++i) {
+            for (int i = 0; i < QPT; ++i) {
                 const float pv[4] = {pa[i].x, pa[i].y, pa[i].z, pa[i].w};
 #pragma unroll
                 for (int c = 0; c < 4; ++c) {
@@ -144,11 +165,11 @@
 
     float* ob = p.o + (long long)b * p.o_bs + h * HD;
 #pragma unroll
-    for (int i = 0; i < 4; ++i) {
+    for (int i = 0; i < QPT; ++i) {
         float l = l_i[i];
 #pragma unroll
         for (int off = 8; off > 0; off >>= 1) l += __shfl_xor_sync(0xffffffffu, l, off);
-        const int q = q0 + ty * 4 + i;
+        const int q = q0 + ty * QPT + i;
         if (q >= p.Tq) continue;
         const float inv = l > 0.f ? 1.0f / l : 0.f;
         *reinterpret_cast<float4*>(ob + (long long)q * p.o_ld + tx * 4) =
@@ -163,13 +184,21 @@
     if (p.B <= 0 || p.Tq <= 0) return 0;
     if (attn_tc_eligible(p, ctx)) return launch_attention_tc(p, stream, ctx);
     static bool configured = false;
+    static int num_sms = 0;
     const int smem_bytes = 4 * HD * LDS_ * (int)sizeof(float);
     if (!configured) {
-        MB_CUDA_CHECK(cudaFuncSetAttribute(attention_kernel, cudaFuncAttributeMaxDynamicSharedMemorySize, smem_bytes));
+        MB_CUDA_CHECK(cudaFuncSetAttribute(attention_kernel<4>, cudaFuncAttributeMaxDynamicSharedMemorySize, smem_bytes));
+        MB_CUDA_CHECK(cudaFuncSetAttribute(attention_kernel<1>, cudaFuncAttributeMaxDynamicSharedMemorySize, smem_bytes));
+        int dev = 0;
+        MB_CUDA_CHECK(cudaGetDevice(&dev));
+        MB_CUDA_CHECK(cudaDeviceGetAttribute(&num_sms, cudaDevAttrMultiProcessorCount, dev));
         configured = true;
     }
-    dim3 grid((p.Tq + TQ - 1) / TQ, p.H, p.B);
-    attention_kernel<<<grid, 256, smem_bytes, stream>>>(p);
+    if ((long long)((p.Tq + TQ - 1) / TQ) * p.H * p.B < num_sms) {
+        attention_kernel<1><<<dim3((p.Tq + 15) / 16, p.H, p.B), 256, smem_bytes, stream>>>(p);
+    } else {
+        attention_kernel<4><<<dim3((p.Tq + TQ - 1) / TQ, p.H, p.B), 256, smem_bytes, stream>>>(p);
+    }
     MB_LAUNCH_CHECK();
     ++g_launch_count;
     return 0;
diff --git a/mapperatorinator_b200/csrc/engine_model.cu b/mapperatorinator_b200/csrc/engine_model.cu
--- a/mapperatorinator_b200/csrc/engine_model.cu
+++ b/mapperatorinator_b200/csrc/engine_model.cu
@@ -1,5 +1,6 @@
 #include <algorithm>
 #include <cstring>
+#include <functional>
 #include <map>
 #include <tuple>
 #include <unordered_map>
@@ -60,6 +61,9 @@
     DevBuf d_attn, d_ticket;
     DevBuf g_state, g_cfg, g_vflags, g_ids, g_prefill_ids, g_keyvalid, g_leftpad, g_rowslot, g_finished, g_lastts, g_lastscores;
     int* h_flag = nullptr;
+    unsigned char* h_stage = nullptr;
+    size_t h_stage_bytes = 0;
+    cudaEvent_t stage_ev = nullptr;
     std::map<std::tuple<int, int, int, int>, cudaGraphExec_t> graphs;
     std::map<std::tuple<int, int, int, int>, long long> graph_nodes;
     bool use_pdl = false;
@@ -181,6 +185,8 @@
     if (m->cap_stream) cudaStreamDestroy(m->cap_stream);
     mel_plan_destroy(m->mel);
     if (m->h_flag) cudaFreeHost(m->h_flag);
+    if (m->h_stage) cudaFreeHost(m->h_stage);
+    if (m->stage_ev) cudaEventDestroy(m->stage_ev);
     delete m;
 }
 
@@ -319,6 +325,12 @@
     MB_TRY(m->g_leftpad.ensure(m->max_rows * sizeof(int)));
     MB_TRY(m->g_rowslot.ensure((size_t)3 * m->max_rows * sizeof(int)));
     MB_TRY(m->g_finished.ensure(m->max_rows));
+    {
+        const size_t tgt = (size_t)m->max_rows * c.tgt_seq_len;
+        m->h_stage_bytes = tgt * 8 * 2 + tgt + (size_t)2 * m->max_rows * 4 + c.vocab_size_in + sizeof(GenState) + sizeof(SampleConfig) + 8 * 16;
+        MB_CUDA_CHECK(cudaMallocHost(&m->h_stage, m->h_stage_bytes));
+        MB_CUDA_CHECK(cudaEventCreateWithFlags(&m->stage_ev, cudaEventDisableTiming));
+    }
     MB_TRY(m->g_lastts.ensure(m->max_rows * sizeof(int)));
     MB_TRY(m->g_lastscores.ensure((size_t)2 * m->max_rows * c.vocab_size_out * sizeof(float)));
     MB_TRY(m->d_x.ensure((size_t)m->max_rows * d * sizeof(float)));
@@ -685,7 +697,8 @@
     return 0;
 }
 
-static int run_megakernel(mb200_model* m, int rows, int B, int n_splits_self, int max_steps, cudaStream_t st) {
+static int run_megakernel(mb200_model* m, int rows, int B, int n_splits_self, int max_steps, cudaStream_t st,
+                          const std::function<int()>& before_sync) {
     auto key = std::make_pair(rows, n_splits_self);
     auto it = m->mega_phases.find(key);
     if (it == m->mega_phases.end()) {
@@ -711,6 +724,7 @@
     MB_CUDA_CHECK(cudaEventRecord(m->mega_ev[1], st));
     MB_CUDA_CHECK(cudaMemcpyAsync(m->h_flag + 1, m->g_megasync.as<int>() + 8, 4, cudaMemcpyDeviceToHost, st));
     MB_CUDA_CHECK(cudaMemcpyAsync(m->h_flag + 3, &m->g_state.as<GenState>()->cur_len, 4, cudaMemcpyDeviceToHost, st));
+    MB_TRY(before_sync());
     MB_CUDA_CHECK(cudaStreamSynchronize(st));
     {
         float ms = 0.f;
@@ -721,7 +735,8 @@
     return 0;
 }
 
-static int run_megakernel2(mb200_model* m, int rows, int B, int n_splits_self, int max_steps, cudaStream_t st) {
+static int run_megakernel2(mb200_model* m, int rows, int B, int n_splits_self, int max_steps, cudaStream_t st,
+                           const std::function<int()>& before_sync) {
     auto key = std::make_tuple(rows, B, n_splits_self);
     auto it = m->mega2_phases.find(key);
     if (it == m->mega2_phases.end()) {
@@ -786,6 +801,7 @@
     MB_CUDA_CHECK(cudaEventRecord(m->mega_ev[1], st));
     MB_CUDA_CHECK(cudaMemcpyAsync(m->h_flag + 1, m->g_megasync.as<int>() + 8, 4, cudaMemcpyDeviceToHost, st));
     MB_CUDA_CHECK(cudaMemcpyAsync(m->h_flag + 3, &m->g_state.as<GenState>()->cur_len, 4, cudaMemcpyDeviceToHost, st));
+    MB_TRY(before_sync());
     MB_CUDA_CHECK(cudaStreamSynchronize(st));
     {
         float ms = 0.f;
@@ -860,17 +876,27 @@
     gs.cur_len = P; gs.prompt_len = P; gs.max_length = gp->max_length; gs.min_new_tokens = gp->min_new_tokens;
     const SampleConfig sc = make_sample_config(gp, B, use_cfg, V, ids_ld);
 
-    MB_CUDA_CHECK(cudaMemcpyAsync(m->g_prefill_ids.p, pre.data(), pre.size() * 8, cudaMemcpyHostToDevice, st));
-    MB_CUDA_CHECK(cudaMemcpyAsync(m->g_ids.p, idsrow.data(), idsrow.size() * 8, cudaMemcpyHostToDevice, st));
-    MB_CUDA_CHECK(cudaMemcpyAsync(m->g_keyvalid.p, kv.data(), kv.size(), cudaMemcpyHostToDevice, st));
-    MB_CUDA_CHECK(cudaMemcpyAsync(m->g_leftpad.p, leftpad.data(), rows * 4, cudaMemcpyHostToDevice, st));
-    MB_CUDA_CHECK(cudaMemcpyAsync(m->g_rowslot.p, rowslot.data(), rows * 4, cudaMemcpyHostToDevice, st));
-    MB_CUDA_CHECK(cudaMemcpyAsync(m->g_vflags.p, vflags, c.vocab_size_in, cudaMemcpyHostToDevice, st));
-    MB_CUDA_CHECK(cudaMemcpyAsync(m->g_state.p, &gs, sizeof(gs), cudaMemcpyHostToDevice, st));
-    MB_CUDA_CHECK(cudaMemcpyAsync(m->g_cfg.p, &sc, sizeof(sc), cudaMemcpyHostToDevice, st));
+    MB_CUDA_CHECK(cudaEventSynchronize(m->stage_ev));
+    size_t stage_off = 0;
+    auto stage = [&](void* dst, const void* src, size_t n) -> int {
+        stage_off = (stage_off + 15) & ~size_t(15);
+        MB_REQUIRE(stage_off + n <= m->h_stage_bytes, "call state exceeds the staging buffer");
+        std::memcpy(m->h_stage + stage_off, src, n);
+        MB_CUDA_CHECK(cudaMemcpyAsync(dst, m->h_stage + stage_off, n, cudaMemcpyHostToDevice, st));
+        stage_off += n;
+        return 0;
+    };
+    MB_TRY(stage(m->g_prefill_ids.p, pre.data(), pre.size() * 8));
+    MB_TRY(stage(m->g_ids.p, idsrow.data(), idsrow.size() * 8));
+    MB_TRY(stage(m->g_keyvalid.p, kv.data(), kv.size()));
+    MB_TRY(stage(m->g_leftpad.p, leftpad.data(), rows * 4));
+    MB_TRY(stage(m->g_rowslot.p, rowslot.data(), rows * 4));
+    MB_TRY(stage(m->g_vflags.p, vflags, c.vocab_size_in));
+    MB_TRY(stage(m->g_state.p, &gs, sizeof(gs)));
+    MB_TRY(stage(m->g_cfg.p, &sc, sizeof(sc)));
+    MB_CUDA_CHECK(cudaEventRecord(m->stage_ev, st));
     MB_CUDA_CHECK(cudaMemsetAsync(m->g_finished.p, 0, m->max_rows, st));
     MB_CUDA_CHECK(cudaMemsetAsync(m->d_ticket.p, 0, (size_t)m->max_rows * m->cfg.heads * sizeof(int), st));
-    MB_CUDA_CHECK(cudaStreamSynchronize(st));
 
     const int chunk = 64;
     const int n_splits_self = self_splits(gp->max_length);
@@ -927,13 +953,19 @@
                        mega2_ksplit_ok(c.ffn_dim, c.d_model, rows, G) && mega2_ksplit_ok(c.d_model, c.ffn_dim, rows, G) &&
                        mega2_ksplit_ok(c.vocab_size_out, c.d_model, rows, G);
         }
-        if (dataflow) MB_TRY(run_megakernel2(m, rows, B, n_splits_self, gp->max_length - (P + 1), st));
-        else MB_TRY(run_megakernel(m, rows, B, n_splits_self, gp->max_length - (P + 1), st));
-        MB_CUDA_CHECK(cudaMemcpyAsync(m->h_flag, &m->g_state.as<GenState>()->cur_len, 4, cudaMemcpyDeviceToHost, st));
-        MB_CUDA_CHECK(cudaStreamSynchronize(st));
-        const int Lm = *m->h_flag;
-        MB_CUDA_CHECK(cudaMemcpy2DAsync(out_ids, (size_t)Lm * 8, m->g_ids.p, (size_t)ids_ld * 8, (size_t)Lm * 8, B, cudaMemcpyDeviceToHost, st));
-        MB_CUDA_CHECK(cudaStreamSynchronize(st));
+        const int Lmax = gp->max_length;
+        MB_REQUIRE((size_t)B * Lmax * 8 <= m->h_stage_bytes, "ids exceed the staging buffer");
+        long long* ids_back = reinterpret_cast<long long*>(m->h_stage);
+        auto read_ids = [&]() -> int {
+            MB_CUDA_CHECK(cudaMemcpy2DAsync(ids_back, (size_t)Lmax * 8, m->g_ids.p, (size_t)ids_ld * 8, (size_t)Lmax * 8, B,
+                                            cudaMemcpyDeviceToHost, st));
+            return 0;
+        };
+        if (dataflow) MB_TRY(run_megakernel2(m, rows, B, n_splits_self, gp->max_length - (P + 1), st, read_ids));
+        else MB_TRY(run_megakernel(m, rows, B, n_splits_self, gp->max_length - (P + 1), st, read_ids));
+        const int Lm = m->h_flag[3];
+        MB_REQUIRE(Lm >= P + 1 && Lm <= Lmax, "megakernel left an out-of-range length");
+        for (int b = 0; b < B; ++b) std::memcpy(out_ids + (size_t)b * Lm, ids_back + (size_t)b * Lmax, (size_t)Lm * 8);
         *out_len = Lm;
         return 0;
     }
diff --git a/mapperatorinator_b200/csrc/gemm.cu b/mapperatorinator_b200/csrc/gemm.cu
--- a/mapperatorinator_b200/csrc/gemm.cu
+++ b/mapperatorinator_b200/csrc/gemm.cu
@@ -9,13 +9,15 @@
 
 constexpr int BM = 128, BN = 128, BK = 16, PAD = 4;
 
+template <int MH>
 __global__ void __launch_bounds__(256, 2) gemm_f32_kernel(GemmParams p) {
-    __shared__ __align__(16) float As[2][BK][BM + PAD];
+    constexpr int TM = 64 * MH;
+    __shared__ __align__(16) float As[2][BK][TM + PAD];
     __shared__ __align__(16) float Bs[2][BK][BN + PAD];
 
     const int tid = threadIdx.x;
     const int tx = tid & 15, ty = tid >> 4;
-    const long long m0 = (long long)blockIdx.y * BM;
+    const long long m0 = (long long)blockIdx.y * TM;
     const int n0 = blockIdx.x * BN;
 
     const int lrow = tid >> 2;
@@ -26,16 +28,16 @@
 #pragma unroll
     for (int h = 0; h < 2; ++h) {
         long long m = m0 + lrow + h * 64;
-        a_ok[h] = m < p.M;
+        a_ok[h] = h < MH && m < p.M;
         a_ptr[h] = a_ok[h] ? p.A.row(p.m_base + m) : p.A.ptr;
         int n = n0 + lrow + h * 64;
         w_ok[h] = n < p.N;
         w_ptr[h] = p.W + (long long)(w_ok[h] ? n : 0) * p.ldw;
     }
 
-    float acc[8][8];
-#pragma unroll
-    for (int i = 0; i < 8; ++i)
+    float acc[4 * MH][8];
+#pragma unroll
+    for (int i = 0; i < 4 * MH; ++i)
 #pragma unroll
         for (int j = 0; j < 8; ++j) acc[i][j] = 0.f;
 
@@ -46,7 +48,7 @@
 #pragma unroll
         for (int h = 0; h < 2; ++h) {
             int k = k_lo_ + k0 + lk;
-            ra[h] = (a_ok[h] && k < k_hi_) ? __ldg(reinterpret_cast<const float4*>(a_ptr[h] + k)) : make_float4(0, 0, 0, 0);
+            if (h < MH) ra[h] = (a_ok[h] && k < k_hi_) ? __ldg(reinterpret_cast<const float4*>(a_ptr[h] + k)) : make_float4(0, 0, 0, 0);
             rw[h] = (w_ok[h] && k < k_hi_) ? __ldg(reinterpret_cast<const float4*>(w_ptr[h] + k)) : make_float4(0, 0, 0, 0);
         }
     };
@@ -54,7 +56,7 @@
 #pragma unroll
         for (int h = 0; h < 2; ++h) {
             int r = lrow + h * 64;
-            As[buf][lk + 0][r] = ra[h].x; As[buf][lk + 1][r] = ra[h].y; As[buf][lk + 2][r] = ra[h].z; As[buf][lk + 3][r] = ra[h].w;
+            if (h < MH) { As[buf][lk + 0][r] = ra[h].x; As[buf][lk + 1][r] = ra[h].y; As[buf][lk + 2][r] = ra[h].z; As[buf][lk + 3][r] = ra[h].w; }
             Bs[buf][lk + 0][r] = rw[h].x; Bs[buf][lk + 1][r] = rw[h].y; Bs[buf][lk + 2][r] = rw[h].z; Bs[buf][lk + 3][r] = rw[h].w;
         }
     };
@@ -71,13 +73,13 @@
 #pragma unroll
         for (int k = 0; k < BK; ++k) {
             float4 a0 = *reinterpret_cast<const float4*>(&As[buf][k][ty * 4]);
-            float4 a1 = *reinterpret_cast<const float4*>(&As[buf][k][64 + ty * 4]);
+            float4 a1 = MH == 2 ? *reinterpret_cast<const float4*>(&As[buf][k][64 * (MH - 1) + ty * 4]) : a0;
             float4 b0 = *reinterpret_cast<const float4*>(&Bs[buf][k][tx * 4]);
             float4 b1 = *reinterpret_cast<const float4*>(&Bs[buf][k][64 + tx * 4]);
             float a[8] = {a0.x, a0.y, a0.z, a0.w, a1.x, a1.y, a1.z, a1.w};
             float b[8] = {b0.x, b0.y, b0.z, b0.w, b1.x, b1.y, b1.z, b1.w};
 #pragma unroll
-            for (int i = 0; i < 8; ++i)
+            for (int i = 0; i < 4 * MH; ++i)
 #pragma unroll
                 for (int j = 0; j < 8; ++j) acc[i][j] = fmaf(a[i], b[j], acc[i][j]);
         }
@@ -89,7 +91,7 @@
 
     if (p.splitk > 1) {
 #pragma unroll
-        for (int i = 0; i < 8; ++i) {
+        for (int i = 0; i < 4 * MH; ++i) {
             long long m = m0 + (i < 4 ? ty * 4 + i : 64 + ty * 4 + (i - 4));
             if (m >= p.M) continue;
             float* wrow = p.splitk_ws + ((long long)blockIdx.z * p.M + m) * p.N;
@@ -104,7 +106,7 @@
         return;
     }
 #pragma unroll
-    for (int i = 0; i < 8; ++i) {
+    for (int i = 0; i < 4 * MH; ++i) {
         long long m = m0 + (i < 4 ? ty * 4 + i : 64 + ty * 4 + (i - 4));
         if (m >= p.M) continue;
         float* crow = p.C.row(p.m_base + m);
@@ -218,9 +220,12 @@
     int kps = 0;
     const int splits = gemm_splits_simt(p.N, p.K, ctx->num_sms, &kps);
     const int tiles_n = (p.N + BN - 1) / BN;
+    const bool half = p.M <= BM;
+    const int tm = half ? BM / 2 : BM;
     if (splits == 1) {
-        dim3 grid(tiles_n, (unsigned)((p.M + BM - 1) / BM));
-        gemm_f32_kernel<<<grid, 256, 0, stream>>>(p);
+        dim3 grid(tiles_n, (unsigned)((p.M + tm - 1) / tm));
+        if (half) gemm_f32_kernel<1><<<grid, 256, 0, stream>>>(p);
+        else gemm_f32_kernel<2><<<grid, 256, 0, stream>>>(p);
         MB_LAUNCH_CHECK();
         ++g_launch_count;
         return 0;
@@ -237,7 +242,9 @@
         q.m_base = p.m_base + m0;
         q.M = (int)std::min<long long>(rows_per_pass, p.M - m0);
         q.splitk_ws = ctx->splitk_ws; q.splitk = splits; q.k_per_split = kps; q.split_mode = 1;
-        gemm_f32_kernel<<<dim3(tiles_n, (unsigned)((q.M + BM - 1) / BM), splits), 256, 0, stream>>>(q);
+        const dim3 grid(tiles_n, (unsigned)((q.M + tm - 1) / tm), splits);
+        if (half) gemm_f32_kernel<1><<<grid, 256, 0, stream>>>(q);
+        else gemm_f32_kernel<2><<<grid, 256, 0, stream>>>(q);
         MB_LAUNCH_CHECK();
         ++g_launch_count;
         const int s = launch_splitk_reduce(q, stream);
diff --git a/mapperatorinator_b200/engine.py b/mapperatorinator_b200/engine.py
--- a/mapperatorinator_b200/engine.py
+++ b/mapperatorinator_b200/engine.py
@@ -59,6 +59,23 @@
     return f
 
 
+class _VflagsCache:
+
+    def __init__(self):
+        self._rows: Dict[tuple, tuple] = {}
+
+    def get(self, layout: TokenLayout, eos_ids: Sequence[int]) -> np.ndarray:
+        key = (id(layout), tuple(eos_ids))
+        hit = self._rows.get(key)
+        if hit is None or hit[0] is not layout:
+            if len(self._rows) >= 64:
+                self._rows.clear()
+            f = build_vflags(layout, eos_ids)
+            f.setflags(write=False)
+            hit = self._rows[key] = (layout, f)
+        return hit[1]
+
+
 class ModelEngine:
 
     def __init__(self, cfg: ModelConfig, state_dict: Dict[str, torch.Tensor], max_windows: int = 32, max_batch: int = 16,
@@ -69,6 +86,7 @@
         self.device = torch.device(device)
         self.lib = _lib.load()
         self.max_windows, self.max_batch = max_windows, max_batch
+        self._vflags = _VflagsCache()
         basis = np.ascontiguousarray(mel_filterbank(cfg.mel) if mel_basis is None else mel_basis, dtype=np.float32)
         cc = _lib.ModelConfigC(cfg.d_model, cfg.encoder_layers, cfg.decoder_layers, cfg.heads, cfg.ffn_dim, cfg.src_seq_len,
                                cfg.tgt_seq_len, cfg.vocab_size_in, cfg.vocab_size_out, _mel_c(cfg.mel), max_windows, max_batch)
@@ -159,7 +177,7 @@
             neg_full[:, :npn.shape[1]] = npn
             neg = np.ascontiguousarray(neg_full)
             nmsk = np.ascontiguousarray(msk.copy() if msk is not None else np.ones_like(ids, dtype=np.uint8))
-        vflags = build_vflags(layout, eos_ids)
+        vflags = self._vflags.get(layout, eos_ids)
         slots_a = np.ascontiguousarray(np.asarray(list(slots), dtype=np.int32))
         assert slots_a.shape[0] == B
         out = np.zeros((B, p.max_length), dtype=np.int64)
@@ -196,7 +214,7 @@
                 npn = np.asarray(torch.as_tensor(neg).detach().cpu().numpy(), dtype=np.int64).reshape(-1)
                 neg_full[:npn.shape[0]] = npn
             params[r] = p
-            vflags[r] = build_vflags(layout, eos_ids)
+            vflags[r] = self._vflags.get(layout, eos_ids)
             prompts.append(ids); negs.append(neg_full)
         if any(cfg_rows) and not all(cfg_rows):
             raise ValueError("classifier-free guidance (negative prompt and cfg_scale > 1) on every request of a ragged call or on none")
@@ -247,7 +265,7 @@
             neg_full[:, :npn.shape[1]] = npn
             neg = np.ascontiguousarray(neg_full)
             nmsk = np.ascontiguousarray(msk.copy() if msk is not None else np.ones_like(ids, dtype=np.uint8))
-        vflags = build_vflags(layout, eos_ids)
+        vflags = self._vflags.get(layout, eos_ids)
         slots_a = np.ascontiguousarray(np.asarray(list(slots), dtype=np.int32))
         assert slots_a.shape[0] == B
         fill = p.pad_token_id if p.pad_token_id else eos_ids[0]
@@ -267,7 +285,7 @@
         p, eos_ids, gk = self._generate_params(layout, generate_kwargs)
         B, L = ids.shape
         a = np.ascontiguousarray(ids.detach().cpu().numpy().astype(np.int64))
-        vflags = build_vflags(layout, eos_ids)
+        vflags = self._vflags.get(layout, eos_ids)
         logits = logits.contiguous().float()
         scores = torch.empty(B, self.cfg.vocab_size_out, device=logits.device, dtype=torch.float32)
         chosen = np.zeros(B, dtype=np.int64)
@@ -284,7 +302,7 @@
         B = BK // num_beams
         a = np.ascontiguousarray(ids.detach().cpu().numpy().astype(np.int64))
         rs = np.ascontiguousarray(run_scores.detach().cpu().numpy().astype(np.float32))
-        vflags = build_vflags(layout, eos_ids)
+        vflags = self._vflags.get(layout, eos_ids)
         logits = logits.contiguous().float()
         lp = torch.empty(BK, self.cfg.vocab_size_out, device=logits.device, dtype=torch.float32)
         out = dict(top=np.zeros(BK, np.int32), parent=np.zeros(BK, np.int32), token=np.zeros(BK, np.int64), score=np.zeros(BK, np.float32),
```
